# schoppmp/linreg-mpc

Measured on AMD Instinct MI355X. Metric: AND-gates/sec (garble+eval) d=500 CGD-15; phase1+2 wall-clock, higher is better.
Workload: dtype int64; 1 GPU; d=500 CGD-15 64-bit p=56, two-party masked input, garbler+evaluator co-located; one system per GPU; d=500, width=64, precision=56

## Files before the change

include/linreg_gc_debug.h:

```cpp
#ifndef LINREG_GC_DEBUG_H
#define LINREG_GC_DEBUG_H
#include "linreg_gc.h"

#ifdef __cplusplus
extern "C" {
#endif

const char *lgc_version(void);
void lgc_trace_set_tag(const char *tag);
void lgc_trace_mark(const char *what);

int lgc_device_warm(int device);
int lgc_preload(int device, int what);

int lgc_solver_get_profile(lgc_solver *s, double *garble_s, double *eval_s, size_t n);

typedef struct {
    uint32_t op, cnt, dst, a, b, c;
    int32_t sa, sb;
    uint64_t step0;
} lgc_record;
typedef struct {
    uint32_t first_rec, nrec;
    uint64_t step0, steps, gates;
    int mac_only;
} lgc_launch;
typedef struct {
    size_t n_records, n_launches;
    uint32_t n_words, n_reveal, in_base, rv_beta, rv_trace, rv_inputs;
    uint64_t total_steps, total_gates, max_launch_steps;
    uint32_t replicas, word_stride, reveal_stride;
    uint32_t shared_end, prefix_launches;
    uint64_t prefix_steps;
    uint64_t total_xors;
} lgc_program_info;
typedef struct lgc_program lgc_program;
int lgc_program_build(lgc_program **out, const lgc_system *sys);
int lgc_program_build_sweep(lgc_program **out, const lgc_system *sys, size_t count, const double *lambdas);
int lgc_program_build_sweep_at(lgc_program **out, const lgc_system *sys, size_t count, const double *lambdas, size_t first);
void lgc_program_destroy(lgc_program *p);
int lgc_program_info_get(const lgc_program *p, lgc_program_info *info);
const lgc_record *lgc_program_records(const lgc_program *p);
const lgc_launch *lgc_program_launches(const lgc_program *p);
int lgc_program_ring_plan(const lgc_program *p, size_t ring_bytes, size_t *ring_bytes_out, size_t *offsets, int64_t *wait_for);

int lgc_reference_gate_count(int algorithm, int width, size_t d, int iterations, uint64_t *gates);

int lgc_solve(int device, const lgc_system *sys, const uint8_t seed[16], const uint64_t *shares,
              int64_t *beta, int64_t *trace, lgc_stats *stats);

int lgc_party_ring_create(lgc_party *p, int nslots, uint8_t handle_out[64], size_t *slot_bytes);
int lgc_party_ring_open(lgc_party *p, const uint8_t handle[64], int nslots, size_t slot_bytes);
int lgc_party_garble_ring_streams(lgc_party *p, int streams);
void lgc_release_cached_memory(void);

void lgc_set_split_kernels(int garbler, int evaluator);

void lgc_set_karatsuba(int on);
void lgc_set_table_ring_slack(size_t bytes);

int lgc_gate_hash_eval(int device, const uint8_t *labels, const uint64_t *tweaks, uint8_t *out, size_t n);

typedef struct {
    uint8_t label[16];
    uint64_t tweak0, stride;
    uint32_t rows, reserved;
} lgc_row_item;
int lgc_row_hash_eval(int device, const lgc_row_item *items, size_t n, uint8_t *out);

int lgc_test_party_garble_ring_stage(lgc_party *p, size_t launch, int stage, int *is_critical_path);
int lgc_test_party_ring_read(lgc_party *p, size_t launch, uint8_t *out, size_t bytes);

#define LGC_LM_AUTO 0
#define LGC_LM_MAC 1
#define LGC_LM_MACK 2
#define LGC_LM_WIDE 3
#define LGC_LM_SPLIT 4
#define LGC_LM_QUAD2 5
int lgc_test_program_create(lgc_program **out, int width, int precision, const lgc_record *records, size_t n_records,
                            const uint32_t *launch_nrec, size_t n_launches, const int *mode_g, const int *mode_e,
                            uint32_t n_inputs, uint32_t n_words, uint32_t n_reveal);
int lgc_test_launch_modes(const lgc_program *p, int *mode_g, int *mode_e, size_t n);
int lgc_test_launch_shape(int mode, int garbler, uint32_t nrec, uint32_t cus, uint32_t *grid, uint32_t *threads,
                          uint32_t *per_wg, uint32_t *max_threads);
typedef struct {
    uint32_t wide_launch, narrow_mac, split_max_recs;
    uint32_t mac_chunk, mac_adapt_lo;
} lgc_test_constants;
void lgc_test_launch_constants(lgc_test_constants *c);
int lgc_test_solver_create(lgc_solver **out, int device, const lgc_program *program, const uint8_t seed[16]);
int lgc_test_solver_reveal(lgc_solver *s, uint64_t *out, size_t n);
int lgc_test_solver_read_words(lgc_solver *s, int garbler, uint32_t first, uint32_t n, uint8_t *out);
int lgc_test_solver_read_tables(lgc_solver *s, size_t launch, uint8_t *out, size_t bytes);

int lgc_test_p1_scan_block(lgc_p1 *h, size_t c0, size_t c1, size_t s0, size_t s1, int with_y, int use_rect, uint64_t *out, double *ms);

int lgc_aes_bench(int device, int waves, int blocks_per_lane, double *rate, uint32_t *check);
int lgc_aes_encrypt(int device, const uint8_t *in, uint8_t *out, size_t n);

#ifdef __cplusplus
}
#endif
#endif
```

linreg-mpc_amd/csrc/gc_engine.hip:

```cpp
#include <hip/hip_runtime.h>
#include <stdarg.h>
#include <stdio.h>
#include <stdlib.h>
#include <string.h>
#include <time.h>

#include <mutex>
#include <string>
#include <utility>
#include <vector>

#include "../../include/linreg_gc.h"
#include "../../include/linreg_gc_sweep.h"
#include "../../include/linreg_gc_debug.h"
#include "../../include/linreg_gc_targets.h"
#include "../../include/linreg_gc_lasso.h"
#include "../../include/linreg_gc_lasso_path.h"
#include "../../include/linreg_gc_lasso_opts.h"
#include "../../include/linreg_gc_lasso_select.h"
#include "../../include/linreg_gc_lasso_cv.h"
#include "../../include/linreg_gc_lasso_cv_se.h"
#include "../../include/linreg_gc_ridge_cv.h"
#include "../../include/linreg_gc_inference.h"
#include "../../include/linreg_gc_scan.h"
// ... 402 lines not shown
                            (size_t)sys->nshares, (unsigned long long)IN, r.scan);
    }
    return LGC_OK;
}

static int validate_path(const BuildRequest &r) {
    if (!r.l1) return lgc_fail(LGC_EINVAL, "null values: a lasso path needs its values of lambda1");
    if (r.l1_count < 1 || r.l1_count > LGC_MAX_L1_PATH)
        return lgc_fail(LGC_EINVAL, "a lasso path takes 1..%d values of lambda1 (got %zu)", LGC_MAX_L1_PATH, r.l1_count);
    if (r.l1_mode != LGC_L1_ABSOLUTE && r.l1_mode != LGC_L1_RATIO)
        return lgc_fail(LGC_EINVAL, "unknown lambda1 mode %d: LGC_L1_ABSOLUTE (0) or LGC_L1_RATIO (1)", r.l1_mode);
    for (size_t l = 0; l < r.l1_count; l++) {
        const double v = r.l1[l];
        if (!std::isfinite(v) || v < 0) return lgc_fail(LGC_EINVAL, "lambda1 path value %zu must be finite and >= 0 (got %g)", l, v);
        if (r.l1_mode == LGC_L1_RATIO && v > 2) return lgc_fail(LGC_EINVAL, "lambda1 ratio %zu is %g: ratios of lambda_max lie in [0, 2]", l, v);
        if (r.l1_mode == LGC_L1_RATIO && r.sys && r.sys->precision >= 0 && r.sys->precision < r.sys->width &&
            std::ldexp(v, r.sys->precision) >= std::ldexp(1.0, r.sys->width - 1))
            return lgc_fail(LGC_EINVAL, "lambda1 ratio %zu is %g: precision %d cannot hold it in a %d-bit word", l, v, r.sys->precision, r.sys->width);
    }
    if (r.sys && r.sys->trace && r.l1_count > 1)
        return lgc_fail(LGC_EINVAL, "trace is for a single lambda1 (its layout has one x per iteration)");
    return LGC_OK;
}

static bool fits_word(double v, int p, int w) {
    const double t = std::ldexp(v, p), top = std::ldexp(1.0, w - 1);
    return t >= -top && t < top;
}

static int validate_opts(const BuildRequest &r) {
    const lgc_lasso_opts &o = *r.opts;
    const int p = r.sys->precision, w = r.sys->width;
    const size_t d = (size_t)r.sys->d;
    for (size_t i = 0; i < d; i++) {
        const double f = o.penalty_factors ? o.penalty_factors[i] : 1.0;
        if (!std::isfinite(f) || f < 0) return lgc_fail(LGC_EINVAL, "penalty factor %zu must be finite and >= 0 (got %g)", i, f);
        const double lo = o.lower ? o.lower[i] : -INFINITY, hi = o.upper ? o.upper[i] : INFINITY;
        if (std::isnan(lo) || std::isnan(hi)) return lgc_fail(LGC_EINVAL, "bound %zu is NaN", i);
        if (lo == INFINITY || hi == -INFINITY)
            return lgc_fail(LGC_EINVAL, "bounds of coordinate %zu are [%g, %g]: no value lies in them", i, lo, hi);
        if (lo > hi) return lgc_fail(LGC_EINVAL, "lower bound %zu is %g, above its upper bound %g", i, lo, hi);
        for (const double v : {lo, hi})
            if (std::isfinite(v) && !fits_word(v, p, w))
                return lgc_fail(LGC_EINVAL, "bound %zu is %g: precision %d cannot hold it in a %d-bit word", i, v, p, w);
        if (!o.penalty_factors) continue;
        for (size_t l = 0; l < r.l1_count; l++) {
            const double v = r.l1[l] * f;
            if (r.l1_mode == LGC_L1_RATIO && !(std::ldexp(v, p) < std::ldexp(1.0, w - 1)))
                return lgc_fail(LGC_EINVAL, "lambda1 ratio %zu times penalty factor %zu is %g: precision %d cannot hold it in a %d-bit word",
                                l, i, v, p, w);
            if (r.l1_mode == LGC_L1_ABSOLUTE && !fits_word(v, p, w))
                return lgc_fail(LGC_EINVAL, "lambda1 %zu times penalty factor %zu is %g: precision %d cannot hold it in a %d-bit word",
                                l, i, v, p, w);
        }
    }
    return LGC_OK;
}

static uint64_t lambda_to_fixed(double lambda, int p, int w) {
    double t = lambda * (double)(1ll << p);
    if (w == 32) {
        if (!(t > -2147483649.0 && t < 2147483648.0)) return (uint64_t)(uint32_t)INT32_MIN;
        return (uint64_t)(uint32_t)(int32_t)t;
    }
    if (!(t >= -9223372036854775808.0 && t < 9223372036854775808.0)) return (uint64_t)INT64_MIN;
    return (uint64_t)(int64_t)t;
}

static int lower(Program &P, const BuildRequest &r, uint64_t cap_steps, size_t merge_hint) {
    const lgc_system *sys = r.sys;
    if (cap_steps) P.cap_steps = cap_steps;
    P.merge_hint = merge_hint;
    const int iters = (sys->algorithm == LGC_ALG_CGD || sys->algorithm == LGC_ALG_LASSO) ? sys->num_iterations : 0;
    Spec s = {sys->algorithm, sys->width, sys->precision, iters, sys->d, sys->nshares, r.targets,
              sys->normalize, sys->reveal_inputs, sys->trace,
              lambda_to_fixed(sys->lambda, sys->precision, sys->width), lambda_to_fixed(r.l1 ? *r.l1 : 0.0, sys->precision, sys->width)};
    std::vector<uint64_t> path;
    if (r.l1_mode != -1) {
        for (size_t l = 0; l < r.l1_count; l++) path.push_back(lambda_to_fixed(r.l1[l], sys->precision, sys->width));
        s.l1_mode = r.l1_mode == LGC_L1_RATIO ? L1_RATIO : L1_ABSOLUTE;
        s.l1_count = r.l1_count;
        s.l1_path = path.data();
    }
    std::vector<uint64_t> coord, lo, hi;
    std::vector<uint8_t> boxed;
    if (r.opts) {
        const lgc_lasso_opts &o = *r.opts;
        const size_t d = (size_t)sys->d;
        bool any = false;
        for (size_t i = 0; i < d; i++)
            any |= (o.penalty_factors && o.penalty_factors[i] != 1.0) || (o.lower && std::isfinite(o.lower[i])) ||
                   (o.upper && std::isfinite(o.upper[i]));
        if (any) {
            const uint64_t wmin = sys->width == 64 ? (uint64_t)INT64_MIN : (uint64_t)(uint32_t)INT32_MIN;
            const uint64_t wmax = sys->width == 64 ? (uint64_t)INT64_MAX : (uint64_t)INT32_MAX;
            for (size_t l = 0; l < r.l1_count; l++)
                for (size_t i = 0; i < d; i++)
                    coord.push_back(lambda_to_fixed(r.l1[l] * (o.penalty_factors ? o.penalty_factors[i] : 1.0), sys->precision, sys->width));
            for (size_t i = 0; i < d; i++) {
                const double a = o.lower ? o.lower[i] : -INFINITY, b = o.upper ? o.upper[i] : INFINITY;
                boxed.push_back(std::isfinite(a) || std::isfinite(b));
                lo.push_back(std::isfinite(a) ? lambda_to_fixed(a, sys->precision, sys->width) : wmin);
                hi.push_back(std::isfinite(b) ? lambda_to_fixed(b, sys->precision, sys->width) : wmax);
            }
            s.l1_coord = coord.data(); s.lo = lo.data(); s.hi = hi.data(); s.boxed = boxed.data();
        }
    }
    s.validate = r.select;
    s.select_reveal = r.reveal;
    s.folds = r.cv ? r.folds : 0;
    s.yy = r.cv && r.se;
    s.cv_rule = s.yy ? r.rule : CV_RULE_MIN;
    if (r.infer) { s.infer = r.reveal; s.resid_fixed = lambda_to_fixed(r.resid_scale, sys->precision, sys->width); }
    if (r.is_scan) {
        s.scan = r.scan; s.scan_bits = r.reveal;
        if (r.reveal & LGC_SCAN_SE) s.resid_fixed = lambda_to_fixed(r.resid_scale, sys->precision, sys->width);
    }
    build_program(P, s);
    if (r.is_scan && P.overflow) return lgc_fail(LGC_EINVAL, "scan too large: the lowered program needs more than 2^31 words");
    if (r.cv && P.overflow) return lgc_fail(LGC_EINVAL, "cross-validation too large: the lowered program needs more than 2^31 words");
    if (r.infer && P.overflow) return lgc_fail(LGC_EINVAL, "inference too large: the lowered program needs more than 2^31 words");
    if (!P.ranges_ok()) return lgc_fail(LGC_EINVAL, "internal: a record of the lowered program lies outside its word file");
    return LGC_OK;
}

static int build_ridge(Program &P, const BuildRequest &r) {
    const lgc_system *sys = r.sys;
    Spec s = {sys->algorithm, sys->width, sys->precision, sys->algorithm == LGC_ALG_CGD ? sys->num_iterations : 0, (size_t)sys->d, (size_t)sys->nshares, 1,
              sys->normalize, 0, 0, 0, 0};
    s.select_reveal = r.reveal;
    std::vector<uint64_t> lf(r.count);
    for (size_t l = 0; l < r.count; l++) lf[l] = lambda_to_fixed(r.lambdas[l], sys->precision, sys->width);
    const int rc = build_ridge_cv(P, s, r.folds, r.count, lf.data(), r.cap_steps);
    if (rc == 1) return lgc_fail(LGC_EINVAL, "ridge cross-validation too large: the lowered program needs more than 2^31 words");
    if (rc) return lgc_fail(LGC_EINVAL, "ridge cross-validation too large: its circuits (more than 65535, or one of more than 2^36 gate steps) do not fit the gate-id stride of a sweep");
    if (!P.ranges_ok()) return lgc_fail(LGC_EINVAL, "internal: a record of the ridge cross-validation lies outside its word file");
    return LGC_OK;
}
static int build(Program &P, const BuildRequest &r) {
    if (r.ridge_cv) return build_ridge(P, r);
    if (!r.sweep) return lower(P, r, r.cap_steps, 1);
    Program base;
    int rcb = lower(base, r, r.cap_steps ? r.cap_steps : kSweepCapSteps, r.count);
    if (rcb) return rcb;
    const size_t count = r.count;
    if ((uint64_t)base.n_words * count >= (1ull << 31)) return lgc_fail(LGC_EINVAL, "sweep too large: %zu circuits x %u words", count, base.n_words);
    std::vector<uint64_t> lf(count);
    for (size_t t = 0; t < count; t++) lf[t] = lambda_to_fixed(r.lambdas[t], r.sys->precision, r.sys->width);
    if (!replicate_program(P, base, count, lf.data(), r.first))
        return lgc_fail(LGC_EINVAL, "sweep too large: a circuit of %llu gate steps (or circuit index %zu) does not fit the gate-id stride of a sweep",
                        (unsigned long long)(base.total_steps - base.prefix_steps), r.first + count);
    if (!P.ranges_ok()) return lgc_fail(LGC_EINVAL, "internal: a record of the merged program lies outside its word file");
    return LGC_OK;
}

static int program_build(lgc_program **out, const BuildRequest &r) {
    int rc = validate(r);
    if (rc) return rc;
    if (!out) return lgc_fail(LGC_EINVAL, r.sweep ? "null argument" : "null out");
    lgc_program *p = new lgc_program();
    rc = build(p->P, r);
    if (rc) { delete p; return rc; }
    *out = p;
    return LGC_OK;
}
static BuildRequest sweep_request(const lgc_system *sys, size_t count, const double *lambdas, size_t first) {
    BuildRequest r = {sys};
    r.sweep = true; r.count = count; r.lambdas = lambdas; r.first = first;
    return r;
}
extern "C" int lgc_program_build(lgc_program **out, const lgc_system *sys) { return program_build(out, {sys}); }
extern "C" int lgc_program_build_lasso(lgc_program **out, const lgc_system *sys, double l1) { return program_build(out, {sys, 1, &l1}); }
static BuildRequest path_request(const lgc_system *sys, size_t count, const double *values, int mode) {
    BuildRequest r = {sys, 1, values};
    r.l1_mode = mode; r.l1_count = count;
    return r;
}
extern "C" int lgc_program_build_lasso_path(lgc_program **out, const lgc_system *sys, size_t count, const double *values, int mode) {
    return program_build(out, path_request(sys, count, values, mode));
}
static BuildRequest opts_request(const lgc_system *sys, const lgc_lasso_opts *opts) {
    BuildRequest r = path_request(sys, opts->l1_count, opts->l1, opts->l1_mode);
    r.opts = opts;
    return r;
}
extern "C" int lgc_program_build_lasso_opts(lgc_program **out, const lgc_system *sys, const lgc_lasso_opts *opts) {
    if (!opts) return lgc_fail(LGC_EINVAL, "null opts");
    return program_build(out, opts_request(sys, opts));
}
static_assert(LGC_SELECT_REVEAL_INDEX == SELECT_REVEAL_INDEX && LGC_SELECT_REVEAL_SCORES == SELECT_REVEAL_SCORES, "LGC_SELECT_REVEAL_* must name the lowering's bits");
static BuildRequest select_request(const lgc_system *sys, const lgc_lasso_opts *opts, int reveal) {
    BuildRequest r = opts_request(sys, opts);
    r.select = true; r.reveal = reveal;
    return r;
}
extern "C" int lgc_program_build_lasso_select(lgc_program **out, const lgc_system *sys, const lgc_lasso_opts *opts, int reveal) {
    if (!opts) return lgc_fail(LGC_EINVAL, "null opts");
    return program_build(out, select_request(sys, opts, reveal));
}
static BuildRequest cv_request(const lgc_system *sys, const lgc_lasso_opts *opts, size_t folds, int reveal) {
    BuildRequest r = opts_request(sys, opts);
    r.cv = true; r.folds = folds; r.reveal = reveal;
    return r;
}
extern "C" int lgc_program_build_lasso_cv(lgc_program **out, const lgc_system *sys, const lgc_lasso_opts *opts, size_t folds, int reveal) {
    if (!opts) return lgc_fail(LGC_EINVAL, "null opts");
    return program_build(out, cv_request(sys, opts, folds, reveal));
}
static_assert(LGC_SELECT_REVEAL_CURVE == SELECT_REVEAL_CURVE && LGC_CV_RULE_MIN == CV_RULE_MIN && LGC_CV_RULE_ONE_SE == CV_RULE_ONE_SE,
              "LGC_SELECT_REVEAL_CURVE and LGC_CV_RULE_* must name the lowering's values");
static BuildRequest cv_se_request(const lgc_system *sys, const lgc_lasso_opts *opts, size_t folds, int reveal, int rule) {
    BuildRequest r = cv_request(sys, opts, folds, reveal);
    r.se = true; r.rule = rule;
    return r;
}
extern "C" int lgc_program_build_lasso_cv_se(lgc_program **out, const lgc_system *sys, const lgc_lasso_opts *opts, size_t folds, int reveal,
                                             int rule) {
    if (!opts) return lgc_fail(LGC_EINVAL, "null opts");
    return program_build(out, cv_se_request(sys, opts, folds, reveal, rule));
}
static BuildRequest ridge_cv_request(const lgc_system *sys, size_t count, const double *lambdas, size_t folds, int reveal) {
    BuildRequest r = {sys};
    r.ridge_cv = true; r.count = count; r.lambdas = lambdas; r.folds = folds; r.reveal = reveal;
    return r;
}
extern "C" int lgc_program_build_ridge_cv(lgc_program **out, const lgc_system *sys, size_t count, const double *lambdas, size_t folds, int reveal) {
    return program_build(out, ridge_cv_request(sys, count, lambdas, folds, reveal));
}
static_assert(LGC_INFER_SE == INFER_SE && LGC_INFER_FIT == INFER_FIT, "LGC_INFER_* must name the lowering's bits");
static BuildRequest inference_request(const lgc_system *sys, double resid_scale, int reveal) {
    BuildRequest r = {sys};
    r.infer = true; r.resid_scale = resid_scale; r.reveal = reveal;
    return r;
}
extern "C" int lgc_program_build_inference(lgc_program **out, const lgc_system *sys, double resid_scale, int reveal) {
    return program_build(out, inference_request(sys, resid_scale, reveal));
}
static_assert(LGC_SCAN_SE == SCAN_SE, "LGC_SCAN_SE must name the lowering's bit");
static BuildRequest scan_request(const lgc_system *sys, size_t M, double resid_scale, int reveal) {
    BuildRequest r = {sys};
    r.is_scan = true; r.scan = M; r.resid_scale = resid_scale; r.reveal = reveal;
    return r;
}
extern "C" int lgc_program_build_scan(lgc_program **out, const lgc_system *sys, size_t M, double resid_scale, int reveal) {
    return program_build(out, scan_request(sys, M, resid_scale, reveal));
}
extern "C" int lgc_program_build_targets(lgc_program **out, const lgc_system *sys, size_t k) { return program_build(out, {sys, k}); }
extern "C" int lgc_program_build_sweep_at(lgc_program **out, const lgc_system *sys, size_t count, const double *lambdas, size_t first) {
    return program_build(out, sweep_request(sys, count, lambdas, first));
}
extern "C" int lgc_program_build_sweep(lgc_program **out, const lgc_system *sys, size_t count, const double *lambdas) {
    return program_build(out, sweep_request(sys, count, lambdas, 0));
}
extern "C" int lgc_program_ring_plan(const lgc_program *p, size_t ring_bytes, size_t *ring_bytes_out, size_t *offsets, int64_t *wait_for) {
    if (!p || !offsets || !wait_for) return lgc_fail(LGC_EINVAL, "null argument");
    std::vector<size_t> off;
    std::vector<int64_t> wait;
    size_t rb = plan_table_ring(p->P, ring_bytes, off, wait);
    if (ring_bytes_out) *ring_bytes_out = rb;
    for (size_t i = 0; i < off.size(); i++) { offsets[i] = off[i]; wait_for[i] = wait[i]; }
    return LGC_OK;
}
extern "C" void lgc_program_destroy(lgc_program *p) { delete p; }
extern "C" int lgc_program_info_get(const lgc_program *p, lgc_program_info *info) {
    if (!p || !info) return lgc_fail(LGC_EINVAL, "null argument");
    const Program &P = p->P;
    info->n_records = P.recs.size();
    info->n_launches = P.launches.size();
    info->n_words = P.n_words;
    info->n_reveal = P.n_reveal;
    info->in_base = P.in_base;
    info->rv_beta = P.rv_beta;
    info->rv_trace = P.rv_trace;
    info->rv_inputs = P.rv_ab;
    info->total_steps = P.total_steps;
    info->total_gates = P.total_gates;
    info->max_launch_steps = P.max_launch_steps;
    info->replicas = P.replicas;
    info->word_stride = P.word_stride;
    info->reveal_stride = P.reveal_stride;
    info->shared_end = P.shared_end;
    info->prefix_launches = P.prefix_launches;
    info->prefix_steps = P.prefix_steps;
    info->total_xors = P.total_xors;
    return LGC_OK;
}
static_assert(sizeof(lgc_record) == sizeof(Rec), "record layout");
extern "C" const lgc_record *lgc_program_records(const lgc_program *p) {
    return reinterpret_cast<const lgc_record *>(p->P.recs.data());
}
extern "C" const lgc_launch *lgc_program_launches(const lgc_program *cp) {
    lgc_program *p = const_cast<lgc_program *>(cp);
    std::vector<lgc_launch> &g_launch_tmp = p->launch_view;
    g_launch_tmp.resize(p->P.launches.size());
    for (size_t i = 0; i < g_launch_tmp.size(); i++) {
        const Launch &L = p->P.launches[i];
        lgc_launch o = {L.first_rec, L.nrec, L.step0, L.steps, L.gates, L.mac_only ? 1 : 0};
        g_launch_tmp[i] = o;
    }
    return g_launch_tmp.data();
}

static_assert(LGC_LM_AUTO == LM_NONE && LGC_LM_MAC == LM_MAC && LGC_LM_MACK == LM_MACK && LGC_LM_WIDE == LM_WIDE &&
              LGC_LM_SPLIT == LM_SPLIT && LGC_LM_QUAD2 == LM_QUAD2, "LGC_LM_* must name the LaunchMode values");
struct FootprintMachine : PlainBackend {
    uint64_t word_end = 0, slot_end = 0;
    void see(uint32_t id) { if ((uint64_t)id + 1 > word_end) word_end = (uint64_t)id + 1; }
    W load(uint32_t id) { see(id); return 0x5a5a5a5a5a5a5a5aull; }
    W load2(uint32_t lo, uint32_t hi) { see(lo); see(hi); return 0x5a5a5a5a5a5a5a5aull; }
    W load2h(uint32_t lo, uint32_t hi) { see(lo); see(hi); return 0x5a5a5a5a5a5a5a5aull; }
    W load2s(uint32_t lo, uint32_t hi, bool) { see(lo); see(hi); return 0x5a5a5a5a5a5a5a5aull; }
    void store(uint32_t id, W) { see(id); }
    void store2(uint32_t lo, uint32_t hi, W) { see(lo); see(hi); }
    void reveal(uint32_t slot, W) { if ((uint64_t)slot + 1 > slot_end) slot_end = (uint64_t)slot + 1; }
};
static bool mode_pairs_steps(LaunchMode m) { return m == LM_SPLIT || m == LM_QUAD2; }
static const char *mode_name(int m) {
    static const char *const n[] = {"auto", "MAC", "MACK", "WIDE", "SPLIT", "QUAD2"};
    return m >= 0 && m <= LM_QUAD2 ? n[m] : "?";
}

extern "C" int lgc_test_program_create(lgc_program **out, int width, int precision, const lgc_record *records, size_t n_records,
                                       const uint32_t *launch_nrec, size_t n_launches, const int *mode_g, const int *mode_e,
                                       uint32_t n_inputs, uint32_t n_words, uint32_t n_reveal) {
    if (!out || !records || !launch_nrec) return lgc_fail(LGC_EINVAL, "null argument");
    if (width != 32 && width != 64) return lgc_fail(LGC_EINVAL, "width must be 32 or 64");
    if (precision < 0 || precision >= width) return lgc_fail(LGC_EINVAL, "precision must satisfy 0 <= p < width");
    if (n_records < 1 || n_launches < 1) return lgc_fail(LGC_EINVAL, "a test program needs at least one launch and one record");
    if (n_words > (1u << 22)) return lgc_fail(LGC_EINVAL, "n_words %u above the test limit of %u", n_words, 1u << 22);
    if ((uint64_t)n_inputs + 1 > n_words) return lgc_fail(LGC_EINVAL, "%u input words at word 1 do not fit n_words = %u", n_inputs, n_words);
    uint64_t sum = 0;
    for (size_t i = 0; i < n_launches; i++) {
        if (launch_nrec[i] < 1) return lgc_fail(LGC_EINVAL, "launch %zu has no records", i);
        sum += launch_nrec[i];
    }
    if (sum != n_records) return lgc_fail(LGC_EINVAL, "the launches hold %llu records, not n_records = %zu", (unsigned long long)sum, n_records);
    for (size_t i = 0; i < n_launches; i++)
        for (int role = 0; role < 2; role++) {
            const int m = role ? (mode_e ? mode_e[i] : 0) : (mode_g ? mode_g[i] : 0);
            if (m < LGC_LM_AUTO || m > LGC_LM_QUAD2) return lgc_fail(LGC_EINVAL, "launch %zu: unknown kernel %d", i, m);
        }
    const Rec *recs = reinterpret_cast<const Rec *>(records);
    for (size_t i = 0; i < n_records; i++) {
        const Rec &r = recs[i];
        if (r.op >= OP_COUNT_) return lgc_fail(LGC_EINVAL, "record %zu: op %u is not an op (OP_COUNT_ = %u)", i, r.op, (unsigned)OP_COUNT_);
        if (width == 64 && r.op == OP_MAC2) return lgc_fail(LGC_EINVAL, "record %zu: OP_MAC2 is a 32-bit op", i);
        if (width == 32 && (r.op == OP_MACK || r.op == OP_HDIFF || r.op == OP_DIVB))
            return lgc_fail(LGC_EINVAL, "record %zu: op %u is a 64-bit op", i, r.op);
        FootprintMachine fm;
        exec_record(fm, r, width, precision);
        if (fm.word_end > n_words)
            return lgc_fail(LGC_EINVAL, "record %zu (op %u): touches word %llu, outside n_words = %u", i, r.op,
                            (unsigned long long)(fm.word_end - 1), n_words);
        if (fm.slot_end > n_reveal)
            return lgc_fail(LGC_EINVAL, "record %zu (op %u): reveals to slot %llu, outside n_reveal = %u", i, r.op,
                            (unsigned long long)(fm.slot_end - 1), n_reveal);
    }
    lgc_program *p = new lgc_program();
    Program &P = p->P;
    P.w = width; P.p = precision;
    P.d = 0; P.T = n_inputs; P.nshares = 1;
    P.in_base = 1; P.shared_end = 1;
    P.n_words = n_words; P.n_reveal = n_reveal;
    size_t next = 0;
    for (size_t i = 0; i < n_launches; i++) {
        P.new_launch();
        for (uint32_t k = 0; k < launch_nrec[i]; k++) P.emit(recs[next++]);
        if (P.launches.size() != i + 1) {
            delete p;
            return lgc_fail(LGC_EINVAL, "launch %zu mixes MAC records (OP_MAC / OP_MAC2 / OP_MACK) with others or with each other, or "
                                        "exceeds the table cap: the lowering would split it", i);
        }
    }
    for (size_t i = 0; i < n_launches; i++) {
        Launch &L = P.launches[i];
        L.force[0] = (uint8_t)(mode_g ? mode_g[i] : 0);
        L.force[1] = (uint8_t)(mode_e ? mode_e[i] : 0);
        for (int role = 0; role < 2; role++) {
            const int m = L.force[role];
            if ((m == LM_MAC || m == LM_MACK) && !L.mac_only) {
                delete p;
                return lgc_fail(LGC_EINVAL, "launch %zu: the %s kernel runs MAC-only launches", i, mode_name(m));
            }
            if ((m == LM_MAC && L.mack) || (m == LM_MACK && !L.mack)) {
                delete p;
                return lgc_fail(LGC_EINVAL, "launch %zu: the %s kernel cannot run %s records", i, mode_name(m),
                                L.mack ? "OP_MACK" : "OP_MAC / OP_MAC2");
            }
        }
        const LaunchMode g = gc_launch_mode(L, true), e = gc_launch_mode(L, false);
        if (mode_pairs_steps(g) != mode_pairs_steps(e)) {
            delete p;
            return lgc_fail(LGC_EINVAL, "launch %zu: garbler %s and evaluator %s number the gate steps differently (kPairSteps)", i,
                            mode_name(g), mode_name(e));
        }
    }
    if (!P.ranges_ok()) {
        delete p;
        return lgc_fail(LGC_EINVAL, "internal: a record of the test program lies outside its word file");
    }
    *out = p;
    return LGC_OK;
}
extern "C" int lgc_test_launch_modes(const lgc_program *p, int *mode_g, int *mode_e, size_t n) {
    if (!p || !mode_g || !mode_e) return lgc_fail(LGC_EINVAL, "null argument");
    if (n != p->P.launches.size()) return lgc_fail(LGC_EINVAL, "n must equal the number of launches (%zu)", p->P.launches.size());
    for (size_t i = 0; i < n; i++) {
        mode_g[i] = gc_launch_mode(p->P.launches[i], true);
        mode_e[i] = gc_launch_mode(p->P.launches[i], false);
    }
    return LGC_OK;
}
extern "C" int lgc_test_launch_shape(int mode, int garbler, uint32_t nrec, uint32_t cus, uint32_t *grid, uint32_t *threads,
                                     uint32_t *per_wg, uint32_t *max_threads) {
    if (!grid || !threads || !per_wg || !max_threads) return lgc_fail(LGC_EINVAL, "null argument");
    if (mode < LGC_LM_MAC || mode > LGC_LM_QUAD2) return lgc_fail(LGC_EINVAL, "unknown kernel %d", mode);
    if (cus < 1) return lgc_fail(LGC_EINVAL, "cus must be >= 1");
    const LaunchShape sh = gc_launch_shape((LaunchMode)mode, garbler != 0, nrec, cus);
    *grid = sh.grid; *threads = sh.threads; *per_wg = sh.per_wg;
    switch (mode) {
    case LM_MAC: *max_threads = garbler ? kTpbMacG : kTpbMacE; break;
    case LM_MACK: *max_threads = garbler ? kTpbMackG : kTpbMackE; break;
    case LM_WIDE: *max_threads = kTpbWide; break;
    case LM_SPLIT: *max_threads = 1024; break;
    default: *max_threads = 256; break;
    }
    return LGC_OK;
}
extern "C" void lgc_test_launch_constants(lgc_test_constants *c) {
    c->wide_launch = kWideLaunch;
    c->narrow_mac = kNarrowMac;
    c->split_max_recs = kSplitMaxRecs;
    c->mac_chunk = kMacChunk;
    c->mac_adapt_lo = kMacAdaptLo;
}

struct lgc_solver {
    lgc_system sys;
    Program P;
    int device;
    Lbl R, seed;
    Lbl *wordsG, *wordsE, *tab;
    uint64_t *decG, *decE, *vals;
    Rec *recs;
    hipStream_t stream, streamE, streamT;
    hipEvent_t ev0, ev1, ev_in;
    size_t ring_bytes;
    size_t tab_alloc_bytes;
    std::vector<size_t> tab_off;
    std::vector<int64_t> tab_wait;
    std::vector<hipEvent_t> evG, evE;
    std::vector<hipEvent_t> evC;
    std::vector<hipEvent_t> evs;
    std::vector<uint64_t> hG, hE;
    std::vector<double> tG, tE;
    std::vector<hipEvent_t> ev_iter;
    std::vector<double> t_iter;
    bool have_shares, ran;
    bool prefix_ready;
    bool prefix_imported = false;
    lgc_stats st;
    lgc_solver() : wordsG(0), wordsE(0), tab(0), decG(0), decE(0), vals(0), recs(0), stream(0), streamE(0), streamT(0), ev0(0), ev1(0), ev_in(0), ring_bytes(0), tab_alloc_bytes(0),
                   have_shares(false), ran(false), prefix_ready(false) { memset(&st, 0, sizeof(st)); }
};

namespace {
struct RingCache {
    std::mutex mu;
    struct Slot { int device; void *ptr; size_t bytes; };
    std::vector<Slot> slots;
    void *take(int device, size_t need, size_t *bytes) {
        std::lock_guard<std::mutex> g(mu);
        for (size_t i = 0; i < slots.size(); i++)
            if (slots[i].device == device && slots[i].bytes >= need) {
                void *p = slots[i].ptr;
                *bytes = slots[i].bytes;
                slots.erase(slots.begin() + (long)i);
                return p;
            }
        return 0;
    }
    void park(int device, void *ptr, size_t bytes) {
        std::lock_guard<std::mutex> g(mu);
        for (size_t i = 0; i < slots.size(); i++)
            if (slots[i].device == device) {
                if (slots[i].bytes >= bytes) { (void)hipFree(ptr); return; }
                (void)hipFree(slots[i].ptr);
                slots[i].ptr = ptr; slots[i].bytes = bytes;
                return;
            }
        Slot n = {device, ptr, bytes};
        slots.push_back(n);
    }
    void release(int device) {
        std::lock_guard<std::mutex> g(mu);
        for (size_t i = 0; i < slots.size();) {
            if (device < 0 || slots[i].device == device) {
                (void)hipSetDevice(slots[i].device);
                (void)hipFree(slots[i].ptr);
                slots.erase(slots.begin() + (long)i);
            } else {
                i++;
            }
        }
    }
};
RingCache &ring_cache() { static RingCache c; return c; }
}

extern "C" void lgc_release_cached_memory(void) { ring_cache().release(-1); }

extern "C" void lgc_solver_destroy(lgc_solver *s) {
    if (!s) return;
    (void)hipSetDevice(s->device);
    if (s->wordsG) (void)hipFree(s->wordsG);
    if (s->wordsE) (void)hipFree(s->wordsE);
    if (s->tab) {
        (void)hipDeviceSynchronize();
        ring_cache().park(s->device, s->tab, s->tab_alloc_bytes);
    }
    if (s->decG) (void)hipFree(s->decG);
    if (s->decE) (void)hipFree(s->decE);
    if (s->vals) (void)hipFree(s->vals);
    if (s->recs) (void)hipFree(s->recs);
    for (size_t i = 0; i < s->evs.size(); i++) (void)hipEventDestroy(s->evs[i]);
    for (size_t i = 0; i < s->ev_iter.size(); i++) (void)hipEventDestroy(s->ev_iter[i]);
    if (s->ev0) (void)hipEventDestroy(s->ev0);
    if (s->ev1) (void)hipEventDestroy(s->ev1);
    for (size_t i = 0; i < s->evG.size(); i++) (void)hipEventDestroy(s->evG[i]);
    for (size_t i = 0; i < s->evE.size(); i++) (void)hipEventDestroy(s->evE[i]);
    for (size_t i = 0; i < s->evC.size(); i++) (void)hipEventDestroy(s->evC[i]);
    if (s->ev_in) (void)hipEventDestroy(s->ev_in);
    if (s->stream) (void)hipStreamDestroy(s->stream);
    if (s->streamE) (void)hipStreamDestroy(s->streamE);
    if (s->streamT) (void)hipStreamDestroy(s->streamT);
    delete s;
}

static int solver_alloc(lgc_solver *s, const uint8_t seed[16], lgc_solver **out);
static int solver_create(lgc_solver **out, int device, const uint8_t seed[16], const BuildRequest &r) {
    int rc = validate(r);
    if (rc) return rc;
    if (!out || !seed) return lgc_fail(LGC_EINVAL, "null argument");
    rc = lgc_need_device(device);
    if (rc) return rc;
    lgc_solver *s = new lgc_solver();
    s->sys = *r.sys;
    s->device = device;
    rc = build(s->P, r);
    if (rc) { delete s; return rc; }
    return solver_alloc(s, seed, out);
}
static int solver_alloc(lgc_solver *s, const uint8_t seed[16], lgc_solver **out) {
    memcpy(&s->seed, seed, 16);
    s->R = derive_R(s->seed);
    const Program &P = s->P;
    size_t wbytes = (size_t)P.n_words * 64 * sizeof(Lbl);
    size_t nin = P.nshares * P.in_words();
#define TRY(x)                                                                                   \
    do {                                                                                         \
        hipError_t e_ = (x);                                                                     \
        if (e_ != hipSuccess) {                                                                  \
            lgc_fail(e_ == hipErrorOutOfMemory ? LGC_ENOMEM : LGC_EHIP, "%s: %s", #x, hipGetErrorString(e_)); \
            lgc_solver_destroy(s);                                                               \
            return e_ == hipErrorOutOfMemory ? LGC_ENOMEM : LGC_EHIP;                            \
        }                                                                                        \
    } while (0)
    TRY(hipStreamCreate(&s->stream));
    TRY(hipStreamCreate(&s->streamE));
    TRY(hipStreamCreate(&s->streamT));
    TRY(hipEventCreate(&s->ev0));
    TRY(hipEventCreate(&s->ev1));
    TRY(hipEventCreateWithFlags(&s->ev_in, hipEventDisableTiming));
    s->ring_bytes = plan_table_ring(P, 0, s->tab_off, s->tab_wait);
    TRY(hipMalloc(&s->wordsG, wbytes));
    TRY(hipMalloc(&s->wordsE, wbytes));
    s->tab = reinterpret_cast<Lbl *>(ring_cache().take(s->device, s->ring_bytes, &s->tab_alloc_bytes));
    if (!s->tab) {
        hipError_t em = hipMalloc(&s->tab, s->ring_bytes);
        if (em == hipErrorOutOfMemory) {
            (void)hipGetLastError();
            ring_cache().release(s->device);
            em = hipMalloc(&s->tab, s->ring_bytes);
        }
        TRY(em);
        s->tab_alloc_bytes = s->ring_bytes;
    }
    TRY(hipMalloc(&s->decG, (P.n_reveal + 1) * sizeof(uint64_t)));
    TRY(hipMalloc(&s->decE, (P.n_reveal + 1) * sizeof(uint64_t)));
    TRY(hipMalloc(&s->vals, nin * sizeof(uint64_t)));
    TRY(hipMalloc(&s->recs, P.recs.size() * sizeof(Rec)));
    TRY(hipMemcpy(s->recs, P.recs.data(), P.recs.size() * sizeof(Rec), hipMemcpyHostToDevice));
#undef TRY
    s->hG.resize(P.n_reveal + 1);
    s->hE.resize(P.n_reveal + 1);
    *out = s;
    return LGC_OK;
}
extern "C" int lgc_solver_create(lgc_solver **out, int device, const lgc_system *sys, const uint8_t seed[16]) {
    return solver_create(out, device, seed, {sys});
}
extern "C" int lgc_solver_create_sweep_at(lgc_solver **out, int device, const lgc_system *sys, const uint8_t seed[16],
                                          size_t count, const double *lambdas, size_t first) {
    return solver_create(out, device, seed, sweep_request(sys, count, lambdas, first));
}
extern "C" int lgc_solver_create_sweep(lgc_solver **out, int device, const lgc_system *sys, const uint8_t seed[16],
                                       size_t count, const double *lambdas) {
    return solver_create(out, device, seed, sweep_request(sys, count, lambdas, 0));
}
extern "C" size_t lgc_solver_num_circuits(const lgc_solver *s) { return s ? (s->P.ridge_cv ? s->P.path : s->P.replicas) : 0; }
extern "C" int lgc_solver_create_ridge_cv(lgc_solver **out, int device, const lgc_system *sys, const uint8_t seed[16], size_t count,
                                          const double *lambdas, size_t folds, int reveal) {
    return solver_create(out, device, seed, ridge_cv_request(sys, count, lambdas, folds, reveal));
}
extern "C" int lgc_solver_create_inference(lgc_solver **out, int device, const lgc_system *sys, const uint8_t seed[16], double resid_scale, int reveal) {
    return solver_create(out, device, seed, inference_request(sys, resid_scale, reveal));
}
extern "C" int lgc_solver_create_scan(lgc_solver **out, int device, const lgc_system *sys, const uint8_t seed[16], size_t M, double resid_scale, int reveal) {
    return solver_create(out, device, seed, scan_request(sys, M, resid_scale, reveal));
}
extern "C" int lgc_solver_create_targets(lgc_solver **out, int device, const lgc_system *sys, const uint8_t seed[16], size_t k) {
    return solver_create(out, device, seed, {sys, k});
}
extern "C" size_t lgc_solver_num_targets(const lgc_solver *s) { return s ? s->P.targets : 0; }
extern "C" int lgc_solver_create_lasso(lgc_solver **out, int device, const lgc_system *sys, const uint8_t seed[16], double l1) {
    return solver_create(out, device, seed, {sys, 1, &l1});
}
extern "C" int lgc_solver_create_lasso_path(lgc_solver **out, int device, const lgc_system *sys, const uint8_t seed[16], size_t count,
                                            const double *values, int mode) {
    return solver_create(out, device, seed, path_request(sys, count, values, mode));
}
extern "C" int lgc_solver_create_lasso_opts(lgc_solver **out, int device, const lgc_system *sys, const uint8_t seed[16],
                                            const lgc_lasso_opts *opts) {
    if (!opts) return lgc_fail(LGC_EINVAL, "null opts");
    return solver_create(out, device, seed, opts_request(sys, opts));
}
extern "C" int lgc_solver_create_lasso_select(lgc_solver **out, int device, const lgc_system *sys, const uint8_t seed[16],
                                              const lgc_lasso_opts *opts, int reveal) {
    if (!opts) return lgc_fail(LGC_EINVAL, "null opts");
    return solver_create(out, device, seed, select_request(sys, opts, reveal));
}
extern "C" int lgc_solver_create_lasso_cv(lgc_solver **out, int device, const lgc_system *sys, const uint8_t seed[16],
                                          const lgc_lasso_opts *opts, size_t folds, int reveal) {
    if (!opts) return lgc_fail(LGC_EINVAL, "null opts");
    return solver_create(out, device, seed, cv_request(sys, opts, folds, reveal));
}
extern "C" int lgc_solver_create_lasso_cv_se(lgc_solver **out, int device, const lgc_system *sys, const uint8_t seed[16],
                                             const lgc_lasso_opts *opts, size_t folds, int reveal, int rule) {
    if (!opts) return lgc_fail(LGC_EINVAL, "null opts");
    return solver_create(out, device, seed, cv_se_request(sys, opts, folds, reveal, rule));
}
extern "C" size_t lgc_solver_num_folds(const lgc_solver *s) { return s ? s->P.folds : 0; }
extern "C" size_t lgc_solver_path_length(const lgc_solver *s) { return s ? s->P.path : 0; }

extern "C" int lgc_test_solver_create(lgc_solver **out, int device, const lgc_program *program, const uint8_t seed[16]) {
    if (!out || !program || !seed) return lgc_fail(LGC_EINVAL, "null argument");
    const int rc = lgc_need_device(device);
    if (rc) return rc;
    lgc_solver *s = new lgc_solver();
    memset(&s->sys, 0, sizeof(s->sys));
    s->sys.width = program->P.w;
    s->sys.precision = program->P.p;
    s->sys.nshares = program->P.nshares;
    s->device = device;
    s->P = program->P;
    return solver_alloc(s, seed, out);
}
extern "C" int lgc_test_solver_reveal(lgc_solver *s, uint64_t *out, size_t n) {
    if (!s || !out) return lgc_fail(LGC_EINVAL, "null argument");
    if (!s->ran) return lgc_fail(LGC_ESTATE, "solver has not run");
    if (n != s->P.n_reveal) return lgc_fail(LGC_EINVAL, "n must equal n_reveal (%u)", s->P.n_reveal);
    const uint64_t m = s->P.w == 64 ? ~0ull : (1ull << s->P.w) - 1;
    for (size_t i = 0; i < n; i++) out[i] = (s->hG[i] ^ s->hE[i]) & m;
    return LGC_OK;
}

extern "C" int lgc_test_solver_read_words(lgc_solver *s, int garbler, uint32_t first, uint32_t n, uint8_t *out) {
    if (!s || !out) return lgc_fail(LGC_EINVAL, "null argument");
    if (!s->ran) return lgc_fail(LGC_ESTATE, "solver has not run");
    if ((uint64_t)first + n > s->P.n_words) return lgc_fail(LGC_EINVAL, "words [%u, %u + %u) lie outside the word file (%u words)", first, first, n, s->P.n_words);
    HIPCHK(hipSetDevice(s->device));
    HIPCHK(hipMemcpy(out, (garbler ? s->wordsG : s->wordsE) + (size_t)first * 64, (size_t)n * 64 * sizeof(Lbl), hipMemcpyDeviceToHost));
    return LGC_OK;
}
extern "C" int lgc_test_solver_read_tables(lgc_solver *s, size_t launch, uint8_t *out, size_t bytes) {
    if (!s || !out) return lgc_fail(LGC_EINVAL, "null argument");
    if (!s->ran) return lgc_fail(LGC_ESTATE, "solver has not run");
    const Program &P = s->P;
    if (launch >= P.launches.size() || bytes != (size_t)P.launches[launch].steps * 2048)
        return lgc_fail(LGC_EINVAL, "launch out of range, or bytes is not 2048 x its gate steps");
    for (size_t k = launch + 1; k < P.launches.size(); k++) {
        const size_t kb = (size_t)P.launches[k].steps * 2048;
        if (kb && s->tab_off[k] < s->tab_off[launch] + bytes && s->tab_off[launch] < s->tab_off[k] + kb)
            return lgc_fail(LGC_ESTATE, "launch %zu has reused the ring region of launch %zu", k, launch);
    }
    HIPCHK(hipSetDevice(s->device));
    HIPCHK(hipMemcpy(out, reinterpret_cast<const uint8_t *>(s->tab) + s->tab_off[launch], bytes, hipMemcpyDeviceToHost));
    return LGC_OK;
}

extern "C" int lgc_solver_set_shares(lgc_solver *s, const uint64_t *shares) {
    if (!s || !shares) return lgc_fail(LGC_EINVAL, "null argument");
    HIPCHK(hipSetDevice(s->device));
    size_t nin = s->P.nshares * s->P.in_words();
    HIPCHK(hipMemcpy(s->vals, shares, nin * sizeof(uint64_t), hipMemcpyHostToDevice));
    s->have_shares = true;
    return LGC_OK;
}

extern "C" int lgc_solver_run(lgc_solver *s, int profile) {
    if (!s) return lgc_fail(LGC_EINVAL, "null solver");
    if (!s->have_shares && !s->prefix_ready)
        return lgc_fail(LGC_ESTATE, s->prefix_imported ? "the imported prefix has been consumed: import again before the next run"
                                                       : "lgc_solver_set_shares has not been called");
    HIPCHK(hipSetDevice(s->device));
    const Program &P = s->P;
    size_t wbytes = (size_t)P.n_words * 64 * sizeof(Lbl);
    size_t nin = P.nshares * P.in_words();
    const size_t nl = P.launches.size();
    size_t need_ev = 3 * nl;
    while (s->evs.size() < need_ev) {
        hipEvent_t e;
        HIPCHK(hipEventCreate(&e));
        s->evs.push_back(e);
    }
    while (s->evG.size() < nl) {
        hipEvent_t a, b;
        HIPCHK(hipEventCreateWithFlags(&a, hipEventDisableTiming));
        s->evG.push_back(a);
        HIPCHK(hipEventCreateWithFlags(&b, hipEventDisableTiming));
        s->evE.push_back(b);
        HIPCHK(hipEventCreateWithFlags(&b, hipEventDisableTiming));
        s->evC.push_back(b);
    }
    hipStream_t sG = s->stream, sE = profile ? s->stream : s->streamE;
// ... 373 lines not shown
```

linreg-mpc_amd/csrc/gc_kernels.h:

```cpp
#pragma once
#include <hip/hip_runtime.h>

#include "gc_device.h"
#include "gc_split.h"
#include "gc_launch.h"

namespace gc {

static inline hipError_t gc_launch_tabfill_impl(const Launch &L, const Lbl *stash, Lbl *tab, Lbl R, hipStream_t st) {
    const uint64_t per = kTpbTabfill / 64;
    uint64_t blocks = (L.steps + per - 1) / per;
    if (blocks > 2048) blocks = 2048;
    hipLaunchKernelGGL((gc_tabfill_kernel<kTpbTabfill>), dim3((unsigned)blocks), dim3(kTpbTabfill), 0, st, stash, tab,
                       (uint32_t)L.steps, L.step0, R);
    return hipGetLastError();
}

template <bool G, int PART>
static inline hipError_t gc_launch_records_impl(LaunchMode m, const Rec *recs, const Launch &L, Lbl *words, uint64_t *dec, Lbl *tab, Lbl R, int w,
                                    int p, hipStream_t st) {
    switch (m) {
    case LM_NONE:
        return hipSuccess;
    case LM_MAC: if constexpr (PART == 0) {
        constexpr int TPB = G ? kTpbMacG : kTpbMacE;
        const LaunchShape sh = gc_launch_shape(m, G, L.nrec, gc_num_cus());
        hipLaunchKernelGGL((gc_mac_kernel<G, TPB>), dim3(sh.grid), dim3(sh.threads), 0, st, recs + L.first_rec, L.nrec, sh.per_wg,
                           words, tab, L.step0, R, w, p);
    } break;
    case LM_MACK: if constexpr (PART == 0) {
        constexpr int TPB = G ? kTpbMackG : kTpbMackE;
        const LaunchShape sh = gc_launch_shape(m, G, L.nrec, gc_num_cus());
        hipLaunchKernelGGL((gc_mack_kernel<G, TPB>), dim3(sh.grid), dim3(sh.threads), 0, st,
                           recs + L.first_rec, L.nrec, sh.per_wg, words, tab, L.step0, R, w, p);
    } break;
    case LM_WIDE: if constexpr (PART == 1) {
        const LaunchShape sh = gc_launch_shape(m, G, L.nrec, gc_num_cus());
        hipLaunchKernelGGL((gc_exec_kernel<G, false, 4, kTpbWide>), dim3(sh.grid), dim3(sh.threads), 0, st,
                           recs + L.first_rec, L.nrec, words, tab, dec, L.step0, R, w, p);
    } break;
    case LM_SPLIT:
        if constexpr (PART == 2) {
            const LaunchShape sh = gc_launch_shape(m, G, L.nrec, gc_num_cus());
            hipLaunchKernelGGL((gc_split_kernel<G>), dim3(sh.grid), dim3(sh.threads), 0, st, recs + L.first_rec, L.nrec, words, tab, dec,
                               L.step0, R, w, p);
        }
        break;
    case LM_QUAD2:
        if constexpr (PART == 3) {
            const LaunchShape sh = gc_launch_shape(m, G, L.nrec, gc_num_cus());
            hipLaunchKernelGGL((gc_exec_kernel<G, true, 2, 256>), dim3(sh.grid), dim3(sh.threads), 0, st, recs + L.first_rec, L.nrec, words,
                               tab, dec, L.step0, R, w, p);
        }
        break;
    }
    return hipGetLastError();
}

}
```

linreg-mpc_amd/csrc/gc_launch.h:

```cpp
#pragma once
#include <hip/hip_runtime.h>

#include <atomic>
#include <cstdlib>
#include <vector>

#include "gc_aes.h"
#include "gc_program.h"

namespace gc {

#ifndef GC_TPB_MACG
#define GC_TPB_MACG 1024
#endif
#ifndef GC_TPB_MACE
#define GC_TPB_MACE 768
#endif
#ifndef GC_TPB_MACKG
#define GC_TPB_MACKG 1024
#endif
#ifndef GC_TPB_MACKE
#define GC_TPB_MACKE 768
#endif
static constexpr int kTpbMacG = GC_TPB_MACG, kTpbMacE = GC_TPB_MACE, kTpbMackG = GC_TPB_MACKG, kTpbMackE = GC_TPB_MACKE;
#ifndef GC_WIDE_LAUNCH
#define GC_WIDE_LAUNCH 520
#endif
static constexpr uint32_t kWideLaunch = GC_WIDE_LAUNCH;
static constexpr int kTpbWide = 768;
static constexpr uint32_t kNarrowMac = 1024;
static constexpr uint32_t kExclusiveMac = 4096;
static constexpr int kTpbTabfill = 1024;
#ifndef GC_SPLIT_MAX_RECS
#define GC_SPLIT_MAX_RECS 256
#endif
static constexpr uint32_t kSplitMaxRecs = GC_SPLIT_MAX_RECS;
inline std::atomic<int> &gc_split_enabled(bool garbler) {
    static std::atomic<int> on[2] = {{1}, {1}};
    return on[garbler ? 0 : 1];
}

static inline unsigned gc_num_cus() {
    static int cus = 0;
    if (!cus) {
        int dev = 0;
        hipDeviceProp_t prop;
        if (hipGetDevice(&dev) == hipSuccess && hipGetDeviceProperties(&prop, dev) == hipSuccess && prop.multiProcessorCount > 0)
            cus = prop.multiProcessorCount;
        else
            cus = 256;
    }
    return (unsigned)cus;
}
static constexpr unsigned kMacAdaptLo = 12, kMacAdaptMaxRounds = 8, kMackAdaptMaxRounds = 3;
static inline unsigned gc_adapt_waves(uint32_t nrec, unsigned lo, unsigned hi, unsigned max_rounds, uint64_t cus) {
    if (((uint64_t)nrec + hi - 1) / hi > (uint64_t)max_rounds * cus || nrec <= cus * lo) return hi;
    unsigned best = hi;
    uint64_t best_cost = ~0ull;
    for (unsigned wv = hi; wv >= lo; wv--) {
        uint64_t wgs = (nrec + wv - 1) / wv, rounds = (wgs + cus - 1) / cus, cost = rounds * wv;
        if (cost < best_cost) { best_cost = cost; best = wv; }
    }
    return best;
}
static constexpr unsigned kMacChunk = 32, kMacChunkMinRounds = 1;
static inline unsigned gc_mac_per_wg(uint32_t nrec, unsigned waves, uint64_t cus) {
    if ((uint64_t)nrec < (uint64_t)kMacChunkMinRounds * cus * waves) return waves;
    uint64_t rounds = ((uint64_t)nrec + cus * waves * kMacChunk / 2) / (cus * waves * kMacChunk);
    if (rounds < 1) rounds = 1;
    const uint64_t wgs = rounds * cus;
    return (unsigned)(((uint64_t)nrec + wgs - 1) / wgs);
}

enum LaunchMode {
    LM_NONE = 0,
    LM_MAC,
    LM_MACK,
    LM_WIDE,
    LM_SPLIT,
    LM_QUAD2
};
static_assert(LM_QUAD2 < 256, "Launch::force holds a LaunchMode in a byte");
static inline LaunchMode gc_launch_mode(const Launch &L, bool garbler) {
    if (L.nrec == 0) return LM_NONE;
    if (L.force[garbler ? 0 : 1]) return (LaunchMode)L.force[garbler ? 0 : 1];
    if (L.mac_only && L.nrec >= kNarrowMac) return L.mack ? LM_MACK : LM_MAC;
    if (L.nrec >= kWideLaunch) return LM_WIDE;
    if (L.nrec <= kSplitMaxRecs && gc_split_enabled(garbler).load(std::memory_order_relaxed)) return LM_SPLIT;
    return LM_QUAD2;
}
struct LaunchShape { uint32_t grid, threads, per_wg; };
static inline LaunchShape gc_launch_shape(LaunchMode m, bool garbler, uint32_t nrec, uint64_t cus) {
    LaunchShape s = {0u, 0u, 0u};
    switch (m) {
    case LM_MAC:
    case LM_MACK: {
        const unsigned tpb = m == LM_MAC ? (garbler ? kTpbMacG : kTpbMacE) : (garbler ? kTpbMackG : kTpbMackE);
        const unsigned per = gc_adapt_waves(nrec, kMacAdaptLo, tpb / 64, m == LM_MAC ? kMacAdaptMaxRounds : kMackAdaptMaxRounds, cus);
        s.per_wg = gc_mac_per_wg(nrec, per, cus);
        s.threads = per * 64;
    } break;
    case LM_WIDE: {
        uint64_t per = ((uint64_t)nrec + cus - 1) / cus;
        if (per > (uint64_t)kTpbWide / 64) per = kTpbWide / 64;
        s.per_wg = (uint32_t)per;
        s.threads = s.per_wg * 64;
    } break;
    case LM_SPLIT: s.per_wg = 1; s.threads = 1024; break;
    case LM_QUAD2: s.per_wg = 1; s.threads = 256; break;
    default: return s;
    }
    s.grid = (uint32_t)(((uint64_t)nrec + s.per_wg - 1) / s.per_wg);
    return s;
}
static inline bool gc_mode_is_crit(LaunchMode m, const Launch &L) { return L.steps != 0 && m == LM_SPLIT; }
hipError_t gc_launch_tabfill(const Launch &L, const Lbl *stash, Lbl *tab, Lbl R, hipStream_t st);
#define GC_KERN_DECL(tag)                                                                                                              \
    hipError_t gc_launch_records_##tag(LaunchMode m, const Rec *recs, const Launch &L, Lbl *words, uint64_t *dec, Lbl *tab, Lbl R, int w, \
                                       int p, hipStream_t st);                                                                         \
    hipError_t gc_kern_touch_##tag(hipStream_t st);
GC_KERN_DECL(g_0) GC_KERN_DECL(g_1) GC_KERN_DECL(g_2) GC_KERN_DECL(g_3) GC_KERN_DECL(e_0) GC_KERN_DECL(e_1) GC_KERN_DECL(e_2) GC_KERN_DECL(e_3)
#undef GC_KERN_DECL
template <bool G>
static inline hipError_t gc_launch_records(LaunchMode m, const Rec *recs, const Launch &L, Lbl *words, uint64_t *dec, Lbl *tab, Lbl R,
                                          int w, int p, hipStream_t st) {
    switch (m) {
    case LM_NONE: return hipSuccess;
    case LM_MAC: case LM_MACK: return G ? gc_launch_records_g_0(m, recs, L, words, dec, tab, R, w, p, st) : gc_launch_records_e_0(m, recs, L, words, dec, tab, R, w, p, st);
    case LM_SPLIT: return G ? gc_launch_records_g_2(m, recs, L, words, dec, tab, R, w, p, st) : gc_launch_records_e_2(m, recs, L, words, dec, tab, R, w, p, st);
    case LM_WIDE: return G ? gc_launch_records_g_1(m, recs, L, words, dec, tab, R, w, p, st) : gc_launch_records_e_1(m, recs, L, words, dec, tab, R, w, p, st);
    default: return G ? gc_launch_records_g_3(m, recs, L, words, dec, tab, R, w, p, st) : gc_launch_records_e_3(m, recs, L, words, dec, tab, R, w, p, st);
    }
}

template <bool G>
static hipError_t gc_preload(const std::vector<Launch> &launches, hipStream_t st) {
    bool need[4] = {false, false, false, false};
    for (const Launch &L : launches) {
        switch (gc_launch_mode(L, G)) {
        case LM_NONE: break;
        case LM_MAC: case LM_MACK: need[0] = true; break;
        case LM_WIDE: need[1] = true; break;
        case LM_SPLIT: need[2] = true; break;
        default: need[3] = true; break;
        }
    }
    hipError_t e = hipSuccess;
    if (need[0] && e == hipSuccess) e = G ? gc_kern_touch_g_0(st) : gc_kern_touch_e_0(st);
    if (need[1] && e == hipSuccess) e = G ? gc_kern_touch_g_1(st) : gc_kern_touch_e_1(st);
    if (need[2] && e == hipSuccess) e = G ? gc_kern_touch_g_2(st) : gc_kern_touch_e_2(st);
    if (need[3] && e == hipSuccess) e = G ? gc_kern_touch_g_3(st) : gc_kern_touch_e_3(st);
    return e;
}

template <bool G>
static hipError_t gc_launch(const Rec *recs, const Launch &L, Lbl *words, uint64_t *dec, Lbl *tab, Lbl R, int w, int p,
                            hipStream_t st, Lbl *stash = 0, int stages = 3, bool *was_crit = 0) {
    const LaunchMode m = gc_launch_mode(L, G);
    const bool crit = G && gc_mode_is_crit(m, L);
    if (was_crit) *was_crit = crit;
    Lbl *rec_tab = (crit && stash) ? stash : tab;
    hipError_t e = hipSuccess;
    if (stages & 1) e = gc_launch_records<G>(m, recs, L, words, dec, rec_tab, R, w, p, st);
    if (e == hipSuccess && crit && (stages & 2)) e = gc_launch_tabfill(L, rec_tab, tab, R, st);
    return e;
}

}
```

linreg-mpc_amd/csrc/gc_split.h:

```cpp
#pragma once
#include "gc_device.h"

namespace gc {

template <int CTRL> __device__ __forceinline__ uint32_t quad_perm(uint32_t v) {
    return (uint32_t)__builtin_amdgcn_mov_dpp((int)v, CTRL, 0xf, 0xf, true);
}

struct HashNoHook { __device__ __forceinline__ void operator()(int) const {} };
template <class F = HashNoHook>
__device__ __forceinline__ uint32_t hash_split(const LdsTab4 &lt, const uint32_t rkl[11], uint32_t x, uint32_t twc, int c, F beside = F()) {
    const uint32_t t = quad_perm<0x4E>(x);
    const uint32_t k = (c < 2) ? (t ^ twc) : (x ^ t);
    uint32_t s = k ^ rkl[0];
#pragma unroll
    for (int rnd = 1; rnd < 10; rnd++) {
        const uint32_t s1 = quad_perm<0x39>(s), s2 = quad_perm<0x4E>(s), s3 = quad_perm<0x93>(s);
        const uint32_t v0 = lt.lkt(0, s, 0), v1 = lt.lkt(1, s1, 1), v2 = lt.lkt(2, s2, 2), v3 = lt.lkt(3, s3, 3);
        beside(rnd);
        s = xor3(xor3(v0, v1, rkl[rnd]), v2, v3);
    }
    const uint32_t s1 = quad_perm<0x39>(s), s2 = quad_perm<0x4E>(s), s3 = quad_perm<0x93>(s);
    const uint32_t v0 = lt.lk(s, 0), v1 = lt.lk(s1, 1), v2 = lt.lk(s2, 2), v3 = lt.lk(s3, 3);
    s = xor3(last_lo(v1, v0), last_hi(v3, v2), rkl[10]);
    return s ^ k;
}

enum {
    kSplitPlane = 72,
    kSplitWord = 4 * kSplitPlane,
    kSplitOp = 0,
    kSplitX = 4 * kSplitWord,
    kSplitKs = 8 * kSplitWord,
    kSplitGs = 16 * kSplitWord,
    kSplitDesc = 20 * kSplitWord,
    kSplitZero = 20 * kSplitWord + 8,
    kSplitWords = 20 * kSplitWord + 16
};

struct SplitDesc {
    uint32_t kind;
    uint64_t act1, act2;
    uint64_t step;
};

struct SplitHashCtx {
    LdsTab4 lt;
    uint32_t rkl[11];
    uint32_t Rq;
    uint32_t *sx;
    __attribute__((address_space(3))) uint32_t *sxl;
    uint32_t *tabw;
    uint64_t launch_step0;
    int wave, lane;
};

__device__ __forceinline__ uint32_t rfl(uint32_t v) { return (uint32_t)__builtin_amdgcn_readfirstlane((int)v); }
__device__ __forceinline__ void st_u32_global(uint32_t *p, uint32_t v) { *(__attribute__((address_space(1))) uint32_t *)p = v; }
__device__ __forceinline__ uint32_t ld_u32_global(const uint32_t *p) { return *(const __attribute__((address_space(1))) uint32_t *)p; }
__device__ __forceinline__ void st_u32_lds(uint32_t *p, uint32_t v) { *(__attribute__((address_space(3))) uint32_t *)p = v; }
__device__ __forceinline__ uint32_t ld_u32_lds(const uint32_t *p) { return *(const __attribute__((address_space(3))) uint32_t *)p; }

__device__ __forceinline__ uint32_t *split_row(const SplitHashCtx &hc, int q, uint64_t st) {
    const int gate = 16 * (hc.wave & 3) + (hc.lane >> 2);
    return hc.tabw + ((st - hc.launch_step0) * 128 + (uint64_t)((q & 1) * 64 + gate)) * 4 + (hc.lane & 3);
}
template <bool GARBLER>
__device__ __forceinline__ void split_hash_core(const SplitHashCtx &hc, int q, uint64_t act, uint64_t st, uint32_t a_op, uint32_t b_op,
                                                uint32_t *xdst, uint32_t tg) {
    const int r = hc.wave & 3, c = hc.lane & 3, gate = 16 * r + (hc.lane >> 2);
    uint32_t *row = split_row(hc, q, st);
    uint32_t *xo = xdst + c * kSplitPlane + gate;
    const uint32_t act16 = (uint32_t)(act >> (16 * r)) & 0xffffu;
    if (act16 == 0) {
        st_u32_lds(xo, 0u);
        if (GARBLER) st_u32_global(row, 0u);
        return;
    }
    const bool on = (act16 >> (hc.lane >> 2)) & 1u;
    const uint32_t v = (q & 1) ? b_op : a_op;
    if (GARBLER) st_u32_global(row, on ? v : 0u);
    const uint32_t colour = quad_perm<0x00>(v) & 1u;
    const uint32_t x = GARBLER ? (v ^ (colour ? hc.Rq : 0u)) : v;
    const uint32_t tlo = ((uint32_t)st << 7) | (uint32_t)(2 * gate + (q & 1)), thi = (uint32_t)(st >> 25);
    const uint32_t twc = (c == 0) ? tlo : (c == 1) ? thi : 0u;
    uint32_t h = hash_split(hc.lt, hc.rkl, x, twc, c);
    if (GARBLER) {
        if (!(q & 1)) h ^= (colour & quad_perm<0x00>(b_op) & 1u) ? hc.Rq : 0u;
    } else {
        h ^= colour ? ((q & 1) ? (tg ^ a_op) : tg) : 0u;
    }
    st_u32_lds(xo, on ? h : 0u);
}

template <bool GARBLER>
__device__ __forceinline__ void split_hash_phase(const SplitHashCtx &hc, const SplitDesc &d) {
    const int q = hc.wave >> 2, r = hc.wave & 3;
    if (d.kind == 1 && q >= 2) return;
    const int c = hc.lane & 3, gate = 16 * r + (hc.lane >> 2);
    const uint32_t *op = hc.sx + kSplitOp + c * kSplitPlane + gate;
    const uint32_t a_op = ld_u32_lds(op + (q & ~1) * kSplitWord), b_op = ld_u32_lds(op + (q | 1) * kSplitWord);
    const uint64_t st = d.step + (uint64_t)(q >> 1);
    const uint32_t tg = GARBLER ? 0u : ld_u32_global(split_row(hc, q, st));
    split_hash_core<GARBLER>(hc, q, (q < 2) ? d.act1 : d.act2, st, a_op, b_op, hc.sx + kSplitX + q * kSplitWord, tg);
}

#ifndef GC_SPLIT_TRACE
#define GC_SPLIT_TRACE 0
#endif
#if GC_SPLIT_TRACE
static __device__ uint64_t g_split_trace[2 * 8192];
static __device__ uint32_t g_split_trace_n[2];
struct SkTrace { bool on; int w; uint32_t i; };
#define SPLIT_STAMP(tag)                                                                                         \
    if (tr.on) {                                                                                                 \
        uint64_t t_;                                                                                             \
        asm volatile("s_memtime %0\n\ts_waitcnt lgkmcnt(0)" : "=s"(t_));                                         \
        if (hc.lane == 0 && tr.i < 8192) g_split_trace[tr.w * 8192 + tr.i] = (t_ << 4) | (uint64_t)(tag);        \
        tr.i++;                                                                                                  \
    }
#define SPLIT_STAMP2(wv, tag)                                                                                    \
    if (GC_SPLIT_TRACE == 2 && blockIdx.x == 0) {                                                                \
        uint64_t t_;                                                                                             \
        asm volatile("s_memtime %0\n\ts_waitcnt lgkmcnt(0)" : "=s"(t_));                                         \
        const uint32_t i_ = g_split_trace_n[wv];                                                                 \
        if ((threadIdx.x & 63) == 0) { if (i_ < 8192) g_split_trace[(wv) * 8192 + i_] = (t_ << 4) | (uint64_t)(tag); g_split_trace_n[wv] = i_ + 1; } \
    }
#else
struct SkTrace {};
#define SPLIT_STAMP(tag)
#define SPLIT_STAMP2(wv, tag)
#endif

typedef __attribute__((address_space(3))) uint32_t lds_u32;

struct SkPtrs {
    const lds_u32 *o0, *o1, *o2;
    const lds_u32 *p0, *p1, *p2;
};

__device__ __forceinline__ int sk_levels(int n) { return n <= 1 ? 0 : 32 - __builtin_clz((uint32_t)(n - 1)); }

__device__ __forceinline__ void sk_words_a(const lds_u32 *sx, int k, int g, int pl, const lds_u32 *&a0, const lds_u32 *&a1) {
    const lds_u32 *opx = sx + kSplitOp + pl, *opy = opx + kSplitWord, *opc = opx + 2 * kSplitWord;
    if (k < 0) { a0 = opx + g; a1 = opc + g; return; }
    const int h = 1 << k, hp = h >> 1;
    const int t = ((g >> k) & 1) ? g : ((g + h) & 63);
    if (k == 0) { a0 = opx + t; a1 = opy + t; return; }
    const lds_u32 *X0 = sx + kSplitKs + ((k & 1) * 4) * kSplitWord + pl, *X1 = X0 + kSplitWord;
    const lds_u32 *Pp = sx + kSplitGs + (((k - 1) & 1) * 2 + 1) * kSplitWord + pl;
    const bool tp = (g >> (k - 1)) & 1;
    const int ti = tp ? t - hp : t;
    a0 = (tp ? X0 : Pp) + ti;
    a1 = tp ? X1 + ti : sx + kSplitZero;
}
__device__ __forceinline__ void sk_words_b(const lds_u32 *sx, int k, int g, int pl, const lds_u32 *&b0, const lds_u32 *&b1, const lds_u32 *&b2) {
    const lds_u32 *opx = sx + kSplitOp + pl, *opy = opx + kSplitWord, *opc = opx + 2 * kSplitWord;
    const lds_u32 *zero = sx + kSplitZero;
    if (k < 0) { b0 = opy + g; b1 = opc + g; b2 = zero; return; }
    const int h = 1 << k, hp = h >> 1;
    const bool up = (g >> k) & 1;
    const int mb = (g & ~(2 * h - 1)) | (h - 1);
    const lds_u32 *X0 = sx + kSplitKs + ((k & 1) * 4) * kSplitWord + pl, *X1 = X0 + kSplitWord;
    if (k == 0) {
        b0 = (up ? X0 : opx) + mb;
        b1 = (up ? X1 : opy) + mb;
        b2 = up ? opc + mb : zero;
        return;
    }
    const lds_u32 *Gp = sx + kSplitGs + (((k - 1) & 1) * 2) * kSplitWord + pl;
    const int mi = up ? mb : ((mb - hp) & 63);
    b0 = X0 + mi;
    b1 = X1 + mi;
    b2 = up ? Gp + mb : zero;
}
template <int Q>
__device__ __forceinline__ void sk_ptrs_own(SkPtrs &r, const lds_u32 *sx, int k, int g, int pl) {
    if (Q == 0) { sk_words_a(sx, k, g, pl, r.o0, r.o1); r.o2 = sx + kSplitZero; }
    else sk_words_b(sx, k, g, pl, r.o0, r.o1, r.o2);
}
template <int Q>
__device__ __forceinline__ void sk_ptrs_oth(SkPtrs &r, const lds_u32 *sx, int k, int g, int plo) {
    if (Q == 0) sk_words_b(sx, k, g, plo, r.p0, r.p1, r.p2);
    else { sk_words_a(sx, k, g, plo, r.p0, r.p1); r.p2 = sx + kSplitZero; }
}

struct SkPlan {
    SkPtrs ptr;
    uint32_t twc;
    bool on;
    bool any;
};
__device__ __forceinline__ bool sk_gate_on(int k, int g, int n) {
    if (k < 0) return g < n;
    const int h = 1 << k;
    return ((g >> k) & 1) ? (g < n) : (g >= 2 * h && g + h < n);
}
template <bool GARBLER, int Q>
__device__ __forceinline__ void sk_plan_part(SkPlan &r, int part, const lds_u32 *sx, int k, int g, int c, int pl, int plo, int n, uint64_t st) {
    constexpr bool kNeedOth = GARBLER ? (Q == 0) : (Q == 1);
    if (part == 0) sk_ptrs_own<Q>(r.ptr, sx, k, g, pl);
    if (part == 1) { if (kNeedOth) sk_ptrs_oth<Q>(r.ptr, sx, k, g, plo); else { r.ptr.p0 = r.ptr.p1 = r.ptr.p2 = sx + kSplitZero; } }
    if (part == 2) {
        const uint32_t tlo = ((uint32_t)st << 7) | (uint32_t)(2 * g + Q), thi = (uint32_t)(st >> 25);
        r.twc = (c == 0) ? tlo : (c == 1) ? thi : 0u;
    }
    if (part == 3) {
        r.on = sk_gate_on(k, g, n);
        r.any = __builtin_amdgcn_ballot_w64(r.on) != 0ull;
    }
}
template <bool GARBLER, int Q>
__device__ __forceinline__ SkPlan sk_plan(const lds_u32 *sx, int k, int g, int c, int pl, int plo, int n, uint64_t st) {
    SkPlan r;
    for (int part = 0; part < 4; part++) sk_plan_part<GARBLER, Q>(r, part, sx, k, g, c, pl, plo, n, st);
    return r;
}

struct SkVals { uint32_t l0, l1, l2, m0, m1, m2; };
template <bool GARBLER, int Q>
__device__ __forceinline__ SkVals sk_load(const SkPtrs &ptr) {
    constexpr bool kNeedOth = GARBLER ? (Q == 0) : (Q == 1);
    SkVals v;
    v.l0 = *ptr.o0; v.l1 = *ptr.o1; v.l2 = (Q == 1) ? *ptr.o2 : 0u;
    v.m0 = v.m1 = v.m2 = 0u;
    if (kNeedOth) { v.m0 = *ptr.p0; v.m1 = *ptr.p1; v.m2 = (Q == 0) ? *ptr.p2 : 0u; }
    return v;
}
template <bool GARBLER, int Q, class F>
__device__ __forceinline__ void sk_finish(const SplitHashCtx &hc, const SkPlan &lv, const SkVals &w, lds_u32 *xo, uint32_t *row, uint32_t tg, F beside) {
    const int c = hc.lane & 3;
    const bool on = lv.on;
    const uint32_t twc = lv.twc;
    if (!lv.any) {
        *xo = 0u;
        if (GARBLER) st_u32_global(row, 0u);
        for (int rnd = 1; rnd < 10; rnd++) beside(rnd);
        return;
    }
    const uint32_t v = xor3(w.l0, w.l1, w.l2);
    if (GARBLER) st_u32_global(row, on ? v : 0u);
    const uint32_t colour = quad_perm<0x00>(v) & 1u;
    const uint32_t x = GARBLER ? (v ^ (colour ? hc.Rq : 0u)) : v;
    uint32_t h = hash_split(hc.lt, hc.rkl, x, twc, c, beside);
    if (GARBLER) {
        if (Q == 0) h ^= (colour & (w.m0 ^ w.m1 ^ w.m2) & 1u) ? hc.Rq : 0u;
    } else {
        h ^= colour ? ((Q == 1) ? (tg ^ xor3(w.m0, w.m1, w.m2)) : tg) : 0u;
    }
    *xo = on ? h : 0u;
}

template <bool GARBLER, int Q>
__device__ __forceinline__ void split_sk_hash(const SplitHashCtx &hc, int n, uint64_t st, const SkVals *pre) {
    const int r = hc.wave & 3, c = hc.lane & 3, g = 16 * r + (hc.lane >> 2);
    SkTrace tr;
    (void)tr;
#if GC_SPLIT_TRACE
    tr.on = GC_SPLIT_TRACE == 1 && blockIdx.x == 0 && (hc.wave == 0 || hc.wave == 4);
    tr.w = hc.wave == 4 ? 1 : 0;
    tr.i = tr.on ? g_split_trace_n[tr.w] : 0u;
    SPLIT_STAMP(1)
#endif
    lds_u32 *sx = hc.sxl;
    const int pl = c * kSplitPlane, plo = GARBLER ? 0 : pl;
    const int L = sk_levels(n);
    uint32_t *row = split_row(hc, Q, st);
    uint32_t tA = 0, tB = 0;
    if (!GARBLER) {
        tA = ld_u32_global(row);
        tB = ld_u32_global(row + (L > 0 ? 512 : 0));
    }
    SkPlan cur = sk_plan<GARBLER, Q>(sx, -1, g, c, pl, plo, n, st), nxt;
    SkVals w = pre ? *pre : sk_load<GARBLER, Q>(cur.ptr);
    sk_finish<GARBLER, Q>(hc, cur, w, sx + kSplitKs + Q * kSplitWord + pl + g, row, tA,
                          [&](int rnd) { if (rnd >= 2 && rnd < 6) sk_plan_part<GARBLER, Q>(nxt, rnd - 2, sx, 0, g, c, pl, plo, n, st + 1); });
    if (!GARBLER) tA = ld_u32_global(row + (L > 1 ? 2 * 512 : 0));
    st += 1;
    row += 512;
    SPLIT_STAMP(2)
    lds_barrier();
    SPLIT_STAMP(3)
    auto level = [&](int k, uint32_t &tg) {
        cur = nxt;
        w = sk_load<GARBLER, Q>(cur.ptr);
        sk_finish<GARBLER, Q>(hc, cur, w, sx + kSplitKs + (((k + 1) & 1) * 4 + Q) * kSplitWord + pl + g, row, tg,
                              [&](int rnd) { if (rnd >= 2 && rnd < 6) sk_plan_part<GARBLER, Q>(nxt, rnd - 2, sx, k + 1, g, c, pl, plo, n, st + 1); });
        if (!GARBLER) tg = ld_u32_global(row + (k + 2 < L ? 2 * 512 : 0));
        SPLIT_STAMP(5)
        st += 1;
        row += 512;
        lds_barrier();
        SPLIT_STAMP(3)
    };
    int k = 0;
    for (; k + 1 < L; k += 2) { level(k, tB); level(k + 1, tA); }
    if (k < L) level(k, tB);
#if GC_SPLIT_TRACE
    if (tr.on && hc.lane == 0) g_split_trace_n[tr.w] = tr.i < 8192 ? tr.i : 8192;
#endif
}

__device__ __forceinline__ void split_sk_side(const SplitHashCtx &hc, int n) {
    const int q = hc.wave >> 2, r = hc.wave & 3, c = hc.lane & 3, g = 16 * r + (hc.lane >> 2);
    lds_u32 *sx = hc.sxl;
    const int pl = c * kSplitPlane;
    const lds_u32 *opx = sx + kSplitOp + pl, *opy = opx + kSplitWord, *opc = opx + 2 * kSplitWord;
    const int L = sk_levels(n);
    lds_barrier();
    for (int k = 0; k < L; k++) {
        if (q == 2) {
            const int h = 1 << k, hp = h >> 1;
            const lds_u32 *X0 = sx + kSplitKs + ((k & 1) * 4) * kSplitWord + pl, *X1 = X0 + kSplitWord;
            const lds_u32 *Gp = sx + kSplitGs + (((k - 1) & 1) * 2) * kSplitWord + pl, *Pp = Gp + kSplitWord;
            lds_u32 *Go = sx + kSplitGs + ((k & 1) * 2) * kSplitWord + pl;
            const uint32_t x0 = X0[g], x1 = X1[g];
            uint32_t Gs, Ps;
            if (k == 0) {
                Gs = x0 ^ x1 ^ opc[g];
                Ps = opx[g] ^ opy[g];
            } else {
                const bool gp = ((g >> (k - 1)) & 1) && g >= h;
                const int gi = gp ? g - hp : g;
                const uint32_t p1 = (gp ? X0 : Pp)[gi], p2 = X1[gi], go = Gp[g];
                Gs = go ^ (((g >> (k - 1)) & 1) ? (x0 ^ x1) : 0u);
                Ps = gp ? (p1 ^ p2) : p1;
            }
            Go[g] = Gs;
            Go[kSplitWord + g] = Ps;
        }
        lds_barrier();
    }
}

template <bool GARBLER>
struct SplitBackend {
    typedef uint32_t W;
    static const bool kPairSteps = true;
    SplitHashCtx hc;
    uint32_t Rc;
    Lbl *words;
    uint64_t *decode;
    uint64_t step;
    int wave, lane;

    __device__ __forceinline__ W zero() const { return 0u; }
    __device__ __forceinline__ bool bit(uint64_t m) const { return __builtin_amdgcn_inverse_ballot_w64(m); }
    __device__ __forceinline__ W rmask(uint64_t m) const { return bit(m) ? Rc : 0u; }
    __device__ __forceinline__ W konst(uint64_t bits) const { return GARBLER ? rmask(bits) : 0u; }
    __device__ __forceinline__ W XOR(W a, W b) const { return a ^ b; }
    __device__ __forceinline__ W NOTm(W a, uint64_t m) const { return GARBLER ? (a ^ rmask(m)) : a; }
    __device__ __forceinline__ W sel(uint64_t m, W a, W b) const { return bit(m) ? a : b; }
    __device__ __forceinline__ W bcast(W a, int src) const { return (uint32_t)__builtin_amdgcn_readlane((int)a, src); }
    __device__ __forceinline__ W bcast2(W a, int r) const { return sel(0xffffffffull, bcast(a, r), bcast(a, 32 + r)); }
    __device__ __forceinline__ W pull(W a, int from, bool ok) const {
        uint32_t v = (uint32_t)__builtin_amdgcn_ds_bpermute((from & 63) << 2, (int)a);
        return ok ? v : 0u;
    }
    __device__ __forceinline__ W bblk(W a, int k) const { const int h = 1 << k; return pull(a, (lane & ~(2 * h - 1)) | (h - 1), true); }
    __device__ __forceinline__ W up1(W a) const { return (uint32_t)__builtin_amdgcn_update_dpp(0, (int)a, 0x138, 0xf, 0xf, true); }
    __device__ __forceinline__ W down1(W a) const { return (uint32_t)__builtin_amdgcn_update_dpp(0, (int)a, 0x130, 0xf, 0xf, true); }
    __device__ __forceinline__ W shl(W a, int k) const {
        if (k == 1) return up1(a);
        if (k == 2) return up1(up1(a));
        return k >= 64 ? 0u : pull(a, lane - k, lane >= k);
    }
    __device__ __forceinline__ W shr(W a, int k) const {
        if (k == 1) return down1(a);
        return k >= 64 ? 0u : pull(a, lane + k, lane + k < 64);
    }

    __device__ __forceinline__ const uint32_t *col(const Lbl *p) const { return reinterpret_cast<const uint32_t *>(p) + wave; }
    __device__ __forceinline__ uint32_t *col(Lbl *p) const { return reinterpret_cast<uint32_t *>(p) + wave; }
    __device__ __forceinline__ W load(uint32_t id) const { return ld_u32_global(col(words + (size_t)id * 64 + lane)); }
    __device__ __forceinline__ W load2(uint32_t lo, uint32_t hi) const {
        return ld_u32_global(col(words + (size_t)(lane < 32 ? lo : hi) * 64 + (lane & 31)));
    }
    __device__ __forceinline__ W load2h(uint32_t lo, uint32_t hi) const {
        return ld_u32_global(col(words + (size_t)(lane < 32 ? lo : hi) * 64 + 32 + (lane & 31)));
    }
    __device__ __forceinline__ W load2s(uint32_t lo, uint32_t hi, bool upper) const { return upper ? load2h(lo, hi) : load2(lo, hi); }
    __device__ __forceinline__ void store(uint32_t id, W v) { st_u32_global(col(words + (size_t)id * 64 + lane), v); }
    __device__ __forceinline__ void store2(uint32_t lo, uint32_t hi, W v) {
        st_u32_global(col(words + (size_t)(lane < 32 ? lo : hi) * 64 + (lane & 31)), v);
    }
    __device__ __forceinline__ void reveal(uint32_t slot, W v) {
        uint64_t m = __ballot(v & 1u);
        if (wave == 0 && lane == 0) decode[slot] = m;
    }

    __device__ __forceinline__ void publish(int k, W v) { st_u32_lds(hc.sx + kSplitOp + k * kSplitWord + wave * kSplitPlane + lane, v); }
    __device__ __forceinline__ W result(int q) const { return ld_u32_lds(hc.sx + kSplitX + q * kSplitWord + wave * kSplitPlane + lane); }
    __device__ __forceinline__ void post(const SplitDesc &d, int n = 0) {
        if (wave == 0 && lane == 0) {
            typedef __attribute__((address_space(3))) gc_u32x4 *lds4;
            gc_u32x4 lo = {d.kind | ((uint32_t)n << 8), (uint32_t)d.step, (uint32_t)(d.step >> 32), (uint32_t)d.act1};
            ((lds4)(hc.sx + kSplitDesc))[0] = lo;
            if (d.kind != 3u) {
                gc_u32x4 hi = {(uint32_t)(d.act1 >> 32), (uint32_t)d.act2, (uint32_t)(d.act2 >> 32), 0u};
                ((lds4)(hc.sx + kSplitDesc))[1] = hi;
            }
        }
    }
    __device__ __forceinline__ W AND(W a, W b, uint64_t act) {
        SplitDesc d = {1u, act, 0ull, step};
        step++;
        publish(0, a);
        publish(1, b);
        post(d);
        lds_barrier();
        split_hash_phase<GARBLER>(hc, d);
        lds_barrier();
        return bit(act) ? (result(0) ^ result(1)) : 0u;
    }
    __device__ __forceinline__ void AND2(W a1, W b1, uint64_t act1, W a2, W b2, uint64_t act2, W &c1, W &c2) {
        SplitDesc d = {2u, act1, act2, step};
        step += 2;
        if (wave == 0) { SPLIT_STAMP2(0, 6) }
        publish(0, a1);
        publish(1, b1);
        publish(2, a2);
        publish(3, b2);
        post(d);
        lds_barrier();
        if (wave == 0) { SPLIT_STAMP2(0, 7) }
        split_hash_phase<GARBLER>(hc, d);
        if (wave == 0) { SPLIT_STAMP2(0, 8) }
        lds_barrier();
        if (wave == 0) { SPLIT_STAMP2(0, 9) }
        c1 = bit(act1) ? (result(0) ^ result(1)) : 0u;
        c2 = bit(act2) ? (result(2) ^ result(3)) : 0u;
        if (wave == 0) { asm volatile("" :: "v"(c1), "v"(c2)); SPLIT_STAMP2(0, 10) }
    }
    __device__ __forceinline__ W add_native(W x, W y, int n, W cinw, W *cout) {
        const int L = sk_levels(n);
        SplitDesc d = {3u, 0ull, 0ull, step};
        const uint64_t st0 = step;
        step += 1 + (uint64_t)L;
        publish(0, x);
        publish(1, y);
        publish(2, cinw);
        post(d, n);
        lds_barrier();
        split_sk_hash<GARBLER, 0>(hc, n, st0, (const SkVals *)0);
        const lds_u32 *sx = hc.sxl;
        const int pl = wave * kSplitPlane;
        const lds_u32 *X0 = sx + kSplitKs + ((L & 1) * 4) * kSplitWord + pl, *X1 = X0 + kSplitWord;
        const lds_u32 *Gp = (L == 0) ? (sx + kSplitOp + 2 * kSplitWord + pl) : (sx + kSplitGs + (((L - 1) & 1) * 2) * kSplitWord + pl);
        const int tm = (lane - 1) & 63;
        const bool xm = (L == 0) || ((tm >> (L - 1)) & 1);
        const uint32_t gm = Gp[tm], x0m = X0[tm], x1m = X1[tm];
        uint32_t co = 0u;
        if (cout) {
            const bool xc = (L == 0) || (((n - 1) >> (L - 1)) & 1);
            co = Gp[n - 1] ^ (xc ? (X0[n - 1] ^ X1[n - 1]) : 0u);
        }
        const uint32_t Gsh = (lane > 0 && lane < n) ? (gm ^ (xm ? (x0m ^ x1m) : 0u)) : 0u;
        if (cout) *cout = co;
        return x ^ y ^ cinw ^ Gsh;
    }
    __device__ __forceinline__ void finish() {
        SplitDesc d = {0u, 0ull, 0ull, 0ull};
        post(d);
        lds_barrier();
    }
};

template <bool GARBLER>
__global__ void __launch_bounds__(1024)
gc_split_kernel(const Rec *recs, uint32_t nrec, Lbl *words, Lbl *tab, uint64_t *decode, uint64_t launch_step0, Lbl R, int w, int p) {
    __shared__ uint32_t lds_te0[2 * kLdsTabWords];
    __shared__ __attribute__((aligned(16))) uint32_t lds_sx[kSplitWords];
    lds_tab4_fill(lds_te0);
    const uint32_t wid = blockIdx.x;
    if (wid >= nrec) return;
    SplitHashCtx hc;
    hc.lt = lds_tab4_make(lds_te0);
    hc.lane = threadIdx.x & 63;
    hc.wave = __builtin_amdgcn_readfirstlane(threadIdx.x >> 6);
    const int c = hc.lane & 3;
#pragma unroll
    for (int k = 0; k < 11; k++) hc.rkl[k] = c_aes.rk[4 * k + c];
    hc.Rq = GARBLER ? (c == 0 ? R.x : c == 1 ? R.y : c == 2 ? R.z : R.w) : 0u;
    hc.sx = lds_sx;
    hc.sxl = (__attribute__((address_space(3))) uint32_t *)lds_sx;
    if (threadIdx.x == 0) lds_sx[kSplitZero] = 0u;
    hc.tabw = reinterpret_cast<uint32_t *>(tab);
    hc.launch_step0 = launch_step0;
    if (hc.wave >= 4) {
        const int q = hc.wave >> 2;
        const int g_ = 16 * (hc.wave & 3) + (hc.lane >> 2), pl_ = c * kSplitPlane;
        SkPtrs first1;
        sk_ptrs_own<1>(first1, hc.sxl, -1, g_, pl_);
        sk_ptrs_oth<1>(first1, hc.sxl, -1, g_, GARBLER ? 0 : pl_);
        for (;;) {
            lds_barrier();
            typedef const __attribute__((address_space(3))) gc_u32x4 *lds4;
            const gc_u32x4 lo = ((lds4)(lds_sx + kSplitDesc))[0];
            SkVals pre;
            if (q == 1) pre = sk_load<GARBLER, 1>(first1);
            SplitDesc d;
            const uint32_t kn = rfl(lo.x);
            d.kind = kn & 0xffu;
            if (d.kind == 0u) return;
            d.step = ((uint64_t)rfl(lo.z) << 32) | rfl(lo.y);
            if (d.kind == 3u) {
                const int n = (int)(kn >> 8);
                if (q == 1) split_sk_hash<GARBLER, 1>(hc, n, d.step, &pre);
                else split_sk_side(hc, n);
                continue;
            }
            const gc_u32x4 hi = ((lds4)(lds_sx + kSplitDesc))[1];
            d.act1 = ((uint64_t)rfl(hi.x) << 32) | rfl(lo.w);
            d.act2 = ((uint64_t)rfl(hi.z) << 32) | rfl(hi.y);
            if (hc.wave == 4) { SPLIT_STAMP2(1, 7) }
            split_hash_phase<GARBLER>(hc, d);
            if (hc.wave == 4) { SPLIT_STAMP2(1, 8) }
            lds_barrier();
            if (hc.wave == 4) { SPLIT_STAMP2(1, 9) }
        }
    }
    SplitBackend<GARBLER> be;
    be.hc = hc;
    be.wave = hc.wave;
    be.lane = hc.lane;
    be.Rc = GARBLER ? (hc.wave == 0 ? R.x : hc.wave == 1 ? R.y : hc.wave == 2 ? R.z : R.w) : 0u;
    be.words = words;
    be.decode = decode;
    Rec r = recs[wid];
    r.op = __builtin_amdgcn_readfirstlane(r.op);
    r.cnt = __builtin_amdgcn_readfirstlane(r.cnt);
    r.dst = __builtin_amdgcn_readfirstlane(r.dst);
    r.a = __builtin_amdgcn_readfirstlane(r.a);
    r.b = __builtin_amdgcn_readfirstlane(r.b);
    r.c = __builtin_amdgcn_readfirstlane(r.c);
    r.sa = __builtin_amdgcn_readfirstlane(r.sa);
    r.sb = __builtin_amdgcn_readfirstlane(r.sb);
    uint32_t s_lo = __builtin_amdgcn_readfirstlane((uint32_t)r.step0);
    uint32_t s_hi = __builtin_amdgcn_readfirstlane((uint32_t)(r.step0 >> 32));
    be.step = ((uint64_t)s_hi << 32) | s_lo;
    exec_record(be, r, w, p);
    be.finish();
}

}
```

linreg-mpc_amd/python/linreg_gc.py:

```python
import ctypes as C
import os
import types

import numpy as np

_HERE = os.path.dirname(os.path.abspath(__file__))
LIB_PATH = os.environ.get("LGC_LIB") or os.path.join(os.path.dirname(_HERE), "csrc", "liblinreg_gc.so")

ALG = {"cholesky": 0, "ldlt": 1, "cgd": 2, "dimcheck": 3,
       "lasso": 4}


class LgcError(RuntimeError):
    def __init__(self, code, msg):
        RuntimeError.__init__(self, "lgc error %d: %s" % (code, msg))
        self.code = code


class System(C.Structure):
    _fields_ = [("d", C.c_size_t), ("width", C.c_int), ("precision", C.c_int), ("algorithm", C.c_int),
                ("num_iterations", C.c_int), ("lam", C.c_double), ("nshares", C.c_size_t),
                ("normalize", C.c_int), ("reveal_inputs", C.c_int), ("trace", C.c_int)]


# ... 914 lines not shown
        _chk(lib().lgc_party_evaluate_ring(self._h, k))

    def garble_ring_begin(self, k):
        _chk(lib().lgc_party_garble_ring_begin(self._h, k))

    def garble_ring_streams(self, n):
        _chk(lib().lgc_party_garble_ring_streams(self._h, n))

    def garble_ring_wait(self, k):
        _chk(lib().lgc_party_garble_ring_wait(self._h, k))

    def test_garble_ring_stage(self, k, stage):
        crit = C.c_int()
        _chk(lib().lgc_test_party_garble_ring_stage(self._h, k, stage, C.byref(crit)))
        return bool(crit.value)

    def test_ring_read(self, k, nbytes):
        out = np.zeros(max(1, nbytes), dtype=np.uint8)
        _chk(lib().lgc_test_party_ring_read(self._h, k, _vp(out), nbytes))
        return out[:nbytes]

    def decode_bits(self):
        out = np.zeros(max(1, self.num_reveal), dtype=np.uint64)
        _chk(lib().lgc_party_decode_bits(self._h, _vp(out)))
        return out

    def finish(self, garbler_dec):
        out = np.zeros(self._req.revealed_shape(), dtype=np.int64)
        trace = np.zeros((1 if self.scan is not None else max(1, self.system.num_iterations), _trace_width(self.system)), dtype=np.int64)
        inputs = np.zeros(self._req.in_words(), dtype=np.int64)
        garbler_dec = np.ascontiguousarray(garbler_dec, dtype=np.uint64)
        _chk(lib().lgc_party_finish(self._h, _vp(garbler_dec), _vp(out), _vp(trace), _vp(inputs)))
        self._result = self._req.split(out)
        return self._result.beta, trace, inputs

    def _need(self, what, name):
        what = "select" if what == "curve" else what
        if self._result is None or getattr(self, what) is None:
            raise LgcError(-1, self._FOLLOWS.get(what) or "%s follows finish() of a model selection" % name)

    def _revealed(self):
        return self._result

    def close(self):
        if self._h:
            lib().lgc_party_destroy(self._h); self._h = None

    def __del__(self):
        try:
            self.close()
        except Exception:
            pass


def share_choice_bits(values, width):
    values = np.ascontiguousarray(values, dtype=np.uint64)
    return ((values[:, None] >> np.arange(width, dtype=np.uint64)[None, :]) & np.uint64(1)).astype(np.uint8).ravel()


class OtSender:

    def __init__(self, delta, seeds, device=0):
        seeds = np.ascontiguousarray(seeds, dtype=np.uint8).reshape(128, 16)
        self._h = C.c_void_p()
        _chk(lib().lgc_ot_sender_create(C.byref(self._h), device, bytes(delta), _vp(seeds)))

    def gilboa(self, b, width, u):
        b = np.ascontiguousarray(b, dtype=np.uint64); npairs, n = b.shape
        y = np.zeros(npairs * n * width, dtype=np.uint64); sh = np.zeros(npairs, dtype=np.uint64)
        _chk(lib().lgc_ot_gilboa_send(self._h, _vp(b), npairs, n, width, _vp(u), _vp(y), _vp(sh)))
        return y, sh

    def set_device_io(self, on):
        _chk(lib().lgc_ot_sender_set_device_io(self._h, 1 if on else 0))

    def gilboa_ptr(self, b_ptr, npairs, n, width, u_ptr, y_ptr, shares_ptr):
        _chk(lib().lgc_ot_gilboa_send(self._h, C.c_void_p(b_ptr), npairs, n, width, C.c_void_p(u_ptr), C.c_void_p(y_ptr), C.c_void_p(shares_ptr)))

    def gilboa_matrix(self, xs, r, width, u):
        xs = np.ascontiguousarray(xs, dtype=np.uint64); rows, s = xs.shape
        y = np.zeros((rows * r * width, s), dtype=np.uint32 if width == 32 else np.uint64); sh = np.zeros((r, s), dtype=np.uint64)
        _chk(lib().lgc_ot_gilboa_matrix_send(self._h, _vp(xs), rows, r, s, width, _vp(u), _vp(y), _vp(sh)))
        return y, sh

    def gilboa_matrix_ptr(self, xs_ptr, rows, r, s, width, u_ptr, y_ptr, shares_ptr):
        _chk(lib().lgc_ot_gilboa_matrix_send(self._h, C.c_void_p(xs_ptr), rows, r, s, width, C.c_void_p(u_ptr), C.c_void_p(y_ptr),
                                             C.c_void_p(shares_ptr)))

    def gilboa_half(self, xs, r, width, u):
        xs = np.ascontiguousarray(xs, dtype=np.uint64); rows, s = xs.shape
        y = np.zeros((rows * r * (width // 2 + 1), s), dtype=np.uint32 if width == 32 else np.uint64); sh = np.zeros((r, s), dtype=np.uint64)
        _chk(lib().lgc_ot_gilboa_half_send(self._h, _vp(xs), rows, r, s, width, _vp(u), _vp(y), _vp(sh)))
        return y, sh

    def gilboa_half_ptr(self, xs_ptr, rows, r, s, width, u_ptr, y_ptr, shares_ptr):
        _chk(lib().lgc_ot_gilboa_half_send(self._h, C.c_void_p(xs_ptr), rows, r, s, width, C.c_void_p(u_ptr), C.c_void_p(y_ptr),
                                           C.c_void_p(shares_ptr)))

    def labels(self, m0, m1, u):
        m0 = np.ascontiguousarray(m0, dtype=np.uint8).reshape(-1, 16); m1 = np.ascontiguousarray(m1, dtype=np.uint8).reshape(-1, 16)
        e = np.zeros((len(m0), 32), dtype=np.uint8)
        _chk(lib().lgc_ot_labels_send(self._h, _vp(m0), _vp(m1), len(m0), _vp(u), _vp(e)))
        return e

    def close(self):
        if self._h:
            lib().lgc_ot_sender_destroy(self._h); self._h = None

    def __del__(self):
        try:
            self.close()
        except Exception:
            pass


class OtReceiver:

    def __init__(self, seeds0, seeds1, device=0):
        seeds0 = np.ascontiguousarray(seeds0, dtype=np.uint8).reshape(128, 16)
        seeds1 = np.ascontiguousarray(seeds1, dtype=np.uint8).reshape(128, 16)
        self._h = C.c_void_p()
        _chk(lib().lgc_ot_receiver_create(C.byref(self._h), device, _vp(seeds0), _vp(seeds1)))

    def gilboa_start(self, a, width):
        a = np.ascontiguousarray(a, dtype=np.uint64); npairs, n = a.shape
        u = np.zeros(lib().lgc_ot_u_bytes(npairs * n * width), dtype=np.uint8)
        _chk(lib().lgc_ot_gilboa_recv_start(self._h, _vp(a), npairs, n, width, _vp(u)))
        if not hasattr(self, "_nps"):
            self._nps = []
        self._nps.append(npairs)
        return u

    def set_device_io(self, on):
        _chk(lib().lgc_ot_receiver_set_device_io(self._h, 1 if on else 0))

    def gilboa_start_ptr(self, a_ptr, npairs, n, width, u_ptr):
        _chk(lib().lgc_ot_gilboa_recv_start(self._h, C.c_void_p(a_ptr), npairs, n, width, C.c_void_p(u_ptr)))

    def gilboa_finish_ptr(self, y_ptr, shares_ptr):
        _chk(lib().lgc_ot_gilboa_recv_finish(self._h, C.c_void_p(y_ptr), C.c_void_p(shares_ptr)))

    def gilboa_finish(self, y):
        if not getattr(self, "_nps", None):
            sh = np.zeros(1, dtype=np.uint64)
            _chk(lib().lgc_ot_gilboa_recv_finish(self._h, _vp(np.ascontiguousarray(y, dtype=np.uint64)), _vp(sh)))
        sh = np.zeros(self._nps.pop(0), dtype=np.uint64)
        _chk(lib().lgc_ot_gilboa_recv_finish(self._h, _vp(np.ascontiguousarray(y, dtype=np.uint64)), _vp(sh)))
        return sh

    def gilboa_matrix_start(self, xr, s, width):
        xr = np.ascontiguousarray(xr, dtype=np.uint64); rows, r = xr.shape
        u = np.zeros(lib().lgc_ot_u_bytes(rows * r * width), dtype=np.uint8)
        _chk(lib().lgc_ot_gilboa_matrix_recv_start(self._h, _vp(xr), rows, r, s, width, _vp(u)))
        if not hasattr(self, "_mats"):
            self._mats = []
        self._mats.append((r, s, width))
        return u

    def gilboa_matrix_finish(self, y):
        if not getattr(self, "_mats", None):
            raise LgcError(-5, "no matrix Gilboa receive was started on this receiver")
        r, s, width = self._mats[0]
        sh = np.zeros((r, s), dtype=np.uint64)
        rc = lib().lgc_ot_gilboa_matrix_recv_finish(self._h, _vp(np.ascontiguousarray(y, dtype=np.uint32 if width == 32 else np.uint64)), _vp(sh))
        if rc != -5:
            self._mats.pop(0)
        _chk(rc)
        return sh

    def gilboa_matrix_start_ptr(self, xr_ptr, rows, r, s, width, u_ptr):
        _chk(lib().lgc_ot_gilboa_matrix_recv_start(self._h, C.c_void_p(xr_ptr), rows, r, s, width, C.c_void_p(u_ptr)))

    def gilboa_matrix_finish_ptr(self, y_ptr, shares_ptr):
        _chk(lib().lgc_ot_gilboa_matrix_recv_finish(self._h, C.c_void_p(y_ptr), C.c_void_p(shares_ptr)))

    def gilboa_half_start(self, xr, s, width):
        xr = np.ascontiguousarray(xr, dtype=np.uint64); rows, r = xr.shape
        u = np.zeros(lib().lgc_ot_u_bytes(rows * r * width), dtype=np.uint8)
        _chk(lib().lgc_ot_gilboa_half_recv_start(self._h, _vp(xr), rows, r, s, width, _vp(u)))
        if not hasattr(self, "_halves"):
            self._halves = []
        self._halves.append((r, s, width))
        return u

    def gilboa_half_finish(self, y):
        if not getattr(self, "_halves", None):
            raise LgcError(-5, "no half-payload Gilboa receive was started on this receiver")
        r, s, width = self._halves[0]
        sh = np.zeros((r, s), dtype=np.uint64)
        rc = lib().lgc_ot_gilboa_half_recv_finish(self._h, _vp(np.ascontiguousarray(y, dtype=np.uint32 if width == 32 else np.uint64)), _vp(sh))
        if rc != -5:
            self._halves.pop(0)
        _chk(rc)
        return sh

    def gilboa_half_start_ptr(self, xr_ptr, rows, r, s, width, u_ptr):
        _chk(lib().lgc_ot_gilboa_half_recv_start(self._h, C.c_void_p(xr_ptr), rows, r, s, width, C.c_void_p(u_ptr)))

    def gilboa_half_finish_ptr(self, y_ptr, shares_ptr):
        _chk(lib().lgc_ot_gilboa_half_recv_finish(self._h, C.c_void_p(y_ptr), C.c_void_p(shares_ptr)))

    def labels_start(self, choice):
        choice = np.ascontiguousarray(choice, dtype=np.uint8)
        self._m = len(choice)
        u = np.zeros(lib().lgc_ot_u_bytes(self._m), dtype=np.uint8)
        _chk(lib().lgc_ot_labels_recv_start(self._h, _vp(choice), self._m, _vp(u)))
        return u

    def labels_finish(self, e):
        out = np.zeros((self._m, 16), dtype=np.uint8)
        _chk(lib().lgc_ot_labels_recv_finish(self._h, _vp(np.ascontiguousarray(e, dtype=np.uint8)), _vp(out)))
        return out

    def close(self):
        if self._h:
            lib().lgc_ot_receiver_destroy(self._h); self._h = None

    def __del__(self):
        try:
            self.close()
        except Exception:
            pass


def release_cached_memory():
    lib().lgc_release_cached_memory()


def set_split_kernels(garbler=True, evaluator=True):
    lib().lgc_set_split_kernels(int(bool(garbler)), int(bool(evaluator)))


def reference_gate_count(algorithm, width, d, iterations=0):
    L = lib()
    L.lgc_reference_gate_count.argtypes = [C.c_int, C.c_int, C.c_size_t, C.c_int, C.POINTER(C.c_uint64)]
    L.lgc_reference_gate_count.restype = C.c_int
    g = C.c_uint64()
    alg = ALG[algorithm] if isinstance(algorithm, str) else int(algorithm)
    return int(g.value) if L.lgc_reference_gate_count(alg, width, d, iterations, C.byref(g)) == 0 else None


def set_karatsuba(on=True):
    lib().lgc_set_karatsuba.argtypes = [C.c_int]; lib().lgc_set_karatsuba.restype = None
    lib().lgc_set_karatsuba(int(bool(on)))


def set_table_ring_slack(nbytes):
    lib().lgc_set_table_ring_slack.argtypes = [C.c_size_t]; lib().lgc_set_table_ring_slack.restype = None
    lib().lgc_set_table_ring_slack(int(nbytes))




def devices_preflight(devices):
    arr = (C.c_int * len(devices))(*[int(v) for v in devices])
    L = lib()
    L.lgc_devices_preflight.argtypes = [C.c_void_p, C.c_size_t]; L.lgc_devices_preflight.restype = C.c_int
    _chk(L.lgc_devices_preflight(arr, len(devices)))


def gate_hash_eval(labels, tweaks, device=0):
    x = np.ascontiguousarray(labels, dtype=np.uint8).reshape(-1, 16)
    t = np.ascontiguousarray(tweaks, dtype=np.uint64).reshape(-1)
    assert len(t) == len(x)
    out = np.zeros_like(x)
    L = lib()
    L.lgc_gate_hash_eval.argtypes = [C.c_int, C.c_void_p, C.c_void_p, C.c_void_p, C.c_size_t]; L.lgc_gate_hash_eval.restype = C.c_int
    _chk(L.lgc_gate_hash_eval(device, x.ctypes.data, t.ctypes.data, out.ctypes.data, len(x)))
    return out


class RowItem(C.Structure):
    _fields_ = [("label", C.c_uint8 * 16), ("tweak0", C.c_uint64), ("stride", C.c_uint64), ("rows", C.c_uint32),
                ("reserved", C.c_uint32)]


def row_hash_eval(items, device=0):
    arr = (RowItem * max(len(items), 1))()
    total = 0
    for it, (label, tweak0, stride, rows) in zip(arr, items):
        it.label[:] = bytes(label)
        it.tweak0, it.stride, it.rows = int(tweak0), int(stride), int(rows)
        total += int(rows)
    out = np.zeros((total, 2, 64, 16), dtype=np.uint8)
    L = lib()
    L.lgc_row_hash_eval.argtypes = [C.c_int, C.c_void_p, C.c_size_t, C.c_void_p]; L.lgc_row_hash_eval.restype = C.c_int
    _chk(L.lgc_row_hash_eval(device, C.cast(arr, C.c_void_p), len(items), out.ctypes.data))
    return out


def aes_bench(waves=8192, blocks_per_lane=256, device=0):
    rate, chk = C.c_double(), C.c_uint32()
    _chk(lib().lgc_aes_bench(device, waves, blocks_per_lane, C.byref(rate), C.byref(chk)))
    return rate.value, chk.value


def aes_encrypt(blocks, device=0):
    blocks = np.ascontiguousarray(blocks, dtype=np.uint8).reshape(-1, 16)
    out = np.empty_like(blocks)
    _chk(lib().lgc_aes_encrypt(device, blocks.ctypes.data_as(C.c_void_p), out.ctypes.data_as(C.c_void_p), len(blocks)))
    return out


LM = {"auto": 0, "mac": 1, "mack": 2, "wide": 3, "split": 4, "quad2": 5}


class LaunchConstants(C.Structure):
    _fields_ = [("wide_launch", C.c_uint32), ("narrow_mac", C.c_uint32), ("split_max_recs", C.c_uint32),
                ("mac_chunk", C.c_uint32), ("mac_adapt_lo", C.c_uint32)]


def _test_fn(name, restype, argtypes):
    fn = getattr(lib(), name)
    fn.restype, fn.argtypes = restype, argtypes
    return fn


def _modes(v, n):
    if v is None:
        return None
    v = [LM[m] if isinstance(m, str) else int(m) for m in v]
    assert len(v) == n, (len(v), n)
    return (C.c_int * n)(*v)


class RecordProgram(Program):

    def __init__(self, width, precision, records, launch_sizes, modes_g=None, modes_e=None, n_inputs=0, n_words=None,
                 n_reveal=0):
        self._h = C.c_void_p()
        recs = (Record * len(records))(*[Record(*(tuple(r) + (0,))) for r in records])
        sizes = (C.c_uint32 * len(launch_sizes))(*[int(n) for n in launch_sizes])
        nl = len(launch_sizes)
        vp, sz, u32 = C.c_void_p, C.c_size_t, C.c_uint32
        fn = _test_fn("lgc_test_program_create", C.c_int,
                      [C.POINTER(vp), C.c_int, C.c_int, vp, sz, vp, sz, vp, vp, u32, u32, u32])
        _chk(fn(C.byref(self._h), width, precision, C.cast(recs, vp), len(records), C.cast(sizes, vp), nl,
                _modes(modes_g, nl), _modes(modes_e, nl), n_inputs, n_words, n_reveal))
        self.info = ProgramInfo()
        _chk(lib().lgc_program_info_get(self._h, C.byref(self.info)))
        self.system = make_system(0, width, precision, nshares=1)

    def modes(self):
        n = self.info.n_launches
        g = (C.c_int * n)(); e = (C.c_int * n)()
        _chk(_test_fn("lgc_test_launch_modes", C.c_int, [C.c_void_p, C.c_void_p, C.c_void_p, C.c_size_t])(self._h, g, e, n))
        return list(g), list(e)


class RecordSolver(Solver):

    def __init__(self, program, seed=b"\x01" * 16, device=0):
        assert len(seed) == 16
        self._h = C.c_void_p()
        self.system = program.system
        self._adopt(_Request(program.system))
        self.count = None
        self._prog = program
        _chk(_test_fn("lgc_test_solver_create", C.c_int, [C.POINTER(C.c_void_p), C.c_int, C.c_void_p, C.c_char_p])(
            C.byref(self._h), device, program._h, seed))

    def set_inputs(self, values):
        v = np.ascontiguousarray(values, dtype=np.uint64)
        _chk(lib().lgc_solver_set_shares(self._h, v.ctypes.data_as(C.c_void_p)))

    def reveal(self):
        n = self._prog.info.n_reveal
        out = np.zeros(n, dtype=np.uint64)
        _chk(_test_fn("lgc_test_solver_reveal", C.c_int, [C.c_void_p, C.c_void_p, C.c_size_t])(self._h, out.ctypes.data_as(C.c_void_p), n))
        return out


    def word_labels(self, garbler, first, n):
        out = np.zeros((n, 64, 16), dtype=np.uint8)
        fn = _test_fn("lgc_test_solver_read_words", C.c_int, [C.c_void_p, C.c_int, C.c_uint32, C.c_uint32, C.c_void_p])
        _chk(fn(self._h, int(bool(garbler)), first, n, out.ctypes.data_as(C.c_void_p)))
        return out

    def tables(self, launch):
        steps = int(self._prog.launches()[launch]["steps"])
        out = np.zeros((steps, 2, 64, 16), dtype=np.uint8)
        fn = _test_fn("lgc_test_solver_read_tables", C.c_int, [C.c_void_p, C.c_size_t, C.c_void_p, C.c_size_t])
        _chk(fn(self._h, launch, out.ctypes.data_as(C.c_void_p), out.nbytes))
        return out


def launch_shape(mode, garbler, nrec, cus):
    u = C.c_uint32
    v = [u(), u(), u(), u()]
    fn = _test_fn("lgc_test_launch_shape", C.c_int, [C.c_int, C.c_int, u, u] + [C.POINTER(u)] * 4)
    _chk(fn(LM[mode] if isinstance(mode, str) else int(mode), int(bool(garbler)), nrec, cus, *[C.byref(x) for x in v]))
    return tuple(x.value for x in v)


def launch_constants():
    c = LaunchConstants()
    _test_fn("lgc_test_launch_constants", None, [C.POINTER(LaunchConstants)])(C.byref(c))
    return {k: getattr(c, k) for k, _ in LaunchConstants._fields_}
```

Before: 16.81 billion AND-gates/s.

## Add SPLIT2 launch mode packing two records per workgroup with per-record LDS barriers

Adds a SPLIT2 launch mode in which one 1024-thread workgroup runs two records, 8 waves each, instead of one record with 16 waves. Each record half synchronises through an LDS atomic counter barrier in place of the workgroup-wide s_barrier, and the sum-hash state stage is folded into the hash rounds so fewer waves cover all four quarters. To fit two records in LDS, the scratch layout shrinks by aliasing the KS region onto the X region. The mode is picked automatically for non-MAC launches with more records than the SPLIT limit (up to twice that) and long step counts. The intent is to halve the grid and improve CU use for these mid-sized critical-path launches, at the cost of spin-wait barriers and more serial work per wave.

```diff
diff --git a/include/linreg_gc_debug.h b/include/linreg_gc_debug.h
--- a/include/linreg_gc_debug.h
+++ b/include/linreg_gc_debug.h
@@ -77,6 +77,7 @@
 #define LGC_LM_WIDE 3
 #define LGC_LM_SPLIT 4
 #define LGC_LM_QUAD2 5
+#define LGC_LM_SPLIT2 20
 int lgc_test_program_create(lgc_program **out, int width, int precision, const lgc_record *records, size_t n_records,
                             const uint32_t *launch_nrec, size_t n_launches, const int *mode_g, const int *mode_e,
                             uint32_t n_inputs, uint32_t n_words, uint32_t n_reveal);
@@ -86,6 +87,7 @@
 typedef struct {
     uint32_t wide_launch, narrow_mac, split_max_recs;
     uint32_t mac_chunk, mac_adapt_lo;
+    uint32_t split2_min_steps;
 } lgc_test_constants;
 void lgc_test_launch_constants(lgc_test_constants *c);
 int lgc_test_solver_create(lgc_solver **out, int device, const lgc_program *program, const uint8_t seed[16]);
diff --git a/linreg-mpc_amd/csrc/gc_engine.hip b/linreg-mpc_amd/csrc/gc_engine.hip
--- a/linreg-mpc_amd/csrc/gc_engine.hip
+++ b/linreg-mpc_amd/csrc/gc_engine.hip
@@ -728,7 +728,7 @@
 }
 
 static_assert(LGC_LM_AUTO == LM_NONE && LGC_LM_MAC == LM_MAC && LGC_LM_MACK == LM_MACK && LGC_LM_WIDE == LM_WIDE &&
-              LGC_LM_SPLIT == LM_SPLIT && LGC_LM_QUAD2 == LM_QUAD2, "LGC_LM_* must name the LaunchMode values");
+              LGC_LM_SPLIT == LM_SPLIT && LGC_LM_QUAD2 == LM_QUAD2 && LGC_LM_SPLIT2 == LM_SPLIT2, "LGC_LM_* must name the LaunchMode values");
 struct FootprintMachine : PlainBackend {
     uint64_t word_end = 0, slot_end = 0;
     void see(uint32_t id) { if ((uint64_t)id + 1 > word_end) word_end = (uint64_t)id + 1; }
@@ -740,10 +740,10 @@
     void store2(uint32_t lo, uint32_t hi, W) { see(lo); see(hi); }
     void reveal(uint32_t slot, W) { if ((uint64_t)slot + 1 > slot_end) slot_end = (uint64_t)slot + 1; }
 };
-static bool mode_pairs_steps(LaunchMode m) { return m == LM_SPLIT || m == LM_QUAD2; }
+static bool mode_pairs_steps(LaunchMode m) { return m == LM_SPLIT || m == LM_SPLIT2 || m == LM_QUAD2; }
 static const char *mode_name(int m) {
     static const char *const n[] = {"auto", "MAC", "MACK", "WIDE", "SPLIT", "QUAD2"};
-    return m >= 0 && m <= LM_QUAD2 ? n[m] : "?";
+    return m == LM_SPLIT2 ? "SPLIT2" : m >= 0 && m <= LM_QUAD2 ? n[m] : "?";
 }
 
 extern "C" int lgc_test_program_create(lgc_program **out, int width, int precision, const lgc_record *records, size_t n_records,
@@ -764,7 +764,7 @@
     for (size_t i = 0; i < n_launches; i++)
         for (int role = 0; role < 2; role++) {
             const int m = role ? (mode_e ? mode_e[i] : 0) : (mode_g ? mode_g[i] : 0);
-            if (m < LGC_LM_AUTO || m > LGC_LM_QUAD2) return lgc_fail(LGC_EINVAL, "launch %zu: unknown kernel %d", i, m);
+            if (!gc_mode_known(m)) return lgc_fail(LGC_EINVAL, "launch %zu: unknown kernel %d", i, m);
         }
     const Rec *recs = reinterpret_cast<const Rec *>(records);
     for (size_t i = 0; i < n_records; i++) {
@@ -840,7 +840,7 @@
 extern "C" int lgc_test_launch_shape(int mode, int garbler, uint32_t nrec, uint32_t cus, uint32_t *grid, uint32_t *threads,
                                      uint32_t *per_wg, uint32_t *max_threads) {
     if (!grid || !threads || !per_wg || !max_threads) return lgc_fail(LGC_EINVAL, "null argument");
-    if (mode < LGC_LM_MAC || mode > LGC_LM_QUAD2) return lgc_fail(LGC_EINVAL, "unknown kernel %d", mode);
+    if (mode == LGC_LM_AUTO || !gc_mode_known(mode)) return lgc_fail(LGC_EINVAL, "unknown kernel %d", mode);
     if (cus < 1) return lgc_fail(LGC_EINVAL, "cus must be >= 1");
     const LaunchShape sh = gc_launch_shape((LaunchMode)mode, garbler != 0, nrec, cus);
     *grid = sh.grid; *threads = sh.threads; *per_wg = sh.per_wg;
@@ -848,7 +848,7 @@
     case LM_MAC: *max_threads = garbler ? kTpbMacG : kTpbMacE; break;
     case LM_MACK: *max_threads = garbler ? kTpbMackG : kTpbMackE; break;
     case LM_WIDE: *max_threads = kTpbWide; break;
-    case LM_SPLIT: *max_threads = 1024; break;
+    case LM_SPLIT: case LM_SPLIT2: *max_threads = 1024; break;
     default: *max_threads = 256; break;
     }
     return LGC_OK;
@@ -857,6 +857,7 @@
     c->wide_launch = kWideLaunch;
     c->narrow_mac = kNarrowMac;
     c->split_max_recs = kSplitMaxRecs;
+    c->split2_min_steps = kSplit2MinSteps;
     c->mac_chunk = kMacChunk;
     c->mac_adapt_lo = kMacAdaptLo;
 }
diff --git a/linreg-mpc_amd/csrc/gc_kernels.h b/linreg-mpc_amd/csrc/gc_kernels.h
--- a/linreg-mpc_amd/csrc/gc_kernels.h
+++ b/linreg-mpc_amd/csrc/gc_kernels.h
@@ -46,6 +46,14 @@
                                L.step0, R, w, p);
         }
         break;
+    case LM_SPLIT2:
+        if constexpr (PART == 2) {
+            const LaunchShape sh = gc_launch_shape(m, G, L.nrec, gc_num_cus());
+            hipLaunchKernelGGL((gc_split_kernel<G, 2>), dim3(sh.grid), dim3(sh.threads), 0, st, recs + L.first_rec, L.nrec, words, tab, dec,
+                               L.step0, R, w, p);
+        }
+        break;
+    case LM_PAIRED: break;
     case LM_QUAD2:
         if constexpr (PART == 3) {
             const LaunchShape sh = gc_launch_shape(m, G, L.nrec, gc_num_cus());
diff --git a/linreg-mpc_amd/csrc/gc_launch.h b/linreg-mpc_amd/csrc/gc_launch.h
--- a/linreg-mpc_amd/csrc/gc_launch.h
+++ b/linreg-mpc_amd/csrc/gc_launch.h
@@ -35,6 +35,14 @@
 #define GC_SPLIT_MAX_RECS 256
 #endif
 static constexpr uint32_t kSplitMaxRecs = GC_SPLIT_MAX_RECS;
+#ifndef GC_SPLIT2_MIN_STEPS
+#define GC_SPLIT2_MIN_STEPS 400
+#endif
+static constexpr uint32_t kSplit2MinSteps = GC_SPLIT2_MIN_STEPS;
+#ifndef GC_SPLIT2_MAX_RECS
+#define GC_SPLIT2_MAX_RECS (2 * GC_SPLIT_MAX_RECS)
+#endif
+static constexpr uint32_t kSplit2MaxRecs = GC_SPLIT2_MAX_RECS;
 inline std::atomic<int> &gc_split_enabled(bool garbler) {
     static std::atomic<int> on[2] = {{1}, {1}};
     return on[garbler ? 0 : 1];
@@ -78,15 +86,21 @@
     LM_MACK,
     LM_WIDE,
     LM_SPLIT,
-    LM_QUAD2
+    LM_QUAD2,
+    LM_PAIRED = 16,
+    LM_SPLIT2 = LM_SPLIT | LM_PAIRED
 };
-static_assert(LM_QUAD2 < 256, "Launch::force holds a LaunchMode in a byte");
+static_assert(LM_SPLIT2 < 256, "Launch::force holds a LaunchMode in a byte");
+static inline bool gc_mode_known(int m) { return (m >= LM_NONE && m <= LM_QUAD2) || m == LM_SPLIT2; }
 static inline LaunchMode gc_launch_mode(const Launch &L, bool garbler) {
     if (L.nrec == 0) return LM_NONE;
     if (L.force[garbler ? 0 : 1]) return (LaunchMode)L.force[garbler ? 0 : 1];
     if (L.mac_only && L.nrec >= kNarrowMac) return L.mack ? LM_MACK : LM_MAC;
+    const bool split_on = gc_split_enabled(garbler).load(std::memory_order_relaxed) != 0;
+    if (split_on && L.nrec > kSplitMaxRecs && L.nrec <= kSplit2MaxRecs && !L.mac_only && L.steps >= (uint64_t)kSplit2MinSteps * L.nrec)
+        return LM_SPLIT2;
     if (L.nrec >= kWideLaunch) return LM_WIDE;
-    if (L.nrec <= kSplitMaxRecs && gc_split_enabled(garbler).load(std::memory_order_relaxed)) return LM_SPLIT;
+    if (L.nrec <= kSplitMaxRecs && split_on) return LM_SPLIT;
     return LM_QUAD2;
 }
 struct LaunchShape { uint32_t grid, threads, per_wg; };
@@ -107,13 +121,14 @@
         s.threads = s.per_wg * 64;
     } break;
     case LM_SPLIT: s.per_wg = 1; s.threads = 1024; break;
+    case LM_SPLIT2: s.per_wg = 2; s.threads = 1024; break;
     case LM_QUAD2: s.per_wg = 1; s.threads = 256; break;
     default: return s;
     }
     s.grid = (uint32_t)(((uint64_t)nrec + s.per_wg - 1) / s.per_wg);
     return s;
 }
-static inline bool gc_mode_is_crit(LaunchMode m, const Launch &L) { return L.steps != 0 && m == LM_SPLIT; }
+static inline bool gc_mode_is_crit(LaunchMode m, const Launch &L) { return L.steps != 0 && (m == LM_SPLIT || m == LM_SPLIT2); }
 hipError_t gc_launch_tabfill(const Launch &L, const Lbl *stash, Lbl *tab, Lbl R, hipStream_t st);
 #define GC_KERN_DECL(tag)                                                                                                              \
     hipError_t gc_launch_records_##tag(LaunchMode m, const Rec *recs, const Launch &L, Lbl *words, uint64_t *dec, Lbl *tab, Lbl R, int w, \
@@ -127,7 +142,7 @@
     switch (m) {
     case LM_NONE: return hipSuccess;
     case LM_MAC: case LM_MACK: return G ? gc_launch_records_g_0(m, recs, L, words, dec, tab, R, w, p, st) : gc_launch_records_e_0(m, recs, L, words, dec, tab, R, w, p, st);
-    case LM_SPLIT: return G ? gc_launch_records_g_2(m, recs, L, words, dec, tab, R, w, p, st) : gc_launch_records_e_2(m, recs, L, words, dec, tab, R, w, p, st);
+    case LM_SPLIT: case LM_SPLIT2: return G ? gc_launch_records_g_2(m, recs, L, words, dec, tab, R, w, p, st) : gc_launch_records_e_2(m, recs, L, words, dec, tab, R, w, p, st);
     case LM_WIDE: return G ? gc_launch_records_g_1(m, recs, L, words, dec, tab, R, w, p, st) : gc_launch_records_e_1(m, recs, L, words, dec, tab, R, w, p, st);
     default: return G ? gc_launch_records_g_3(m, recs, L, words, dec, tab, R, w, p, st) : gc_launch_records_e_3(m, recs, L, words, dec, tab, R, w, p, st);
     }
@@ -141,7 +156,7 @@
         case LM_NONE: break;
         case LM_MAC: case LM_MACK: need[0] = true; break;
         case LM_WIDE: need[1] = true; break;
-        case LM_SPLIT: need[2] = true; break;
+        case LM_SPLIT: case LM_SPLIT2: need[2] = true; break;
         default: need[3] = true; break;
         }
     }
diff --git a/linreg-mpc_amd/csrc/gc_split.h b/linreg-mpc_amd/csrc/gc_split.h
--- a/linreg-mpc_amd/csrc/gc_split.h
+++ b/linreg-mpc_amd/csrc/gc_split.h
@@ -31,11 +31,12 @@
     kSplitWord = 4 * kSplitPlane,
     kSplitOp = 0,
     kSplitX = 4 * kSplitWord,
-    kSplitKs = 8 * kSplitWord,
-    kSplitGs = 16 * kSplitWord,
-    kSplitDesc = 20 * kSplitWord,
-    kSplitZero = 20 * kSplitWord + 8,
-    kSplitWords = 20 * kSplitWord + 16
+    kSplitKs = kSplitX,
+    kSplitGs = 8 * kSplitWord,
+    kSplitDesc = 12 * kSplitWord,
+    kSplitZero = 12 * kSplitWord + 8,
+    kSplitBar = 12 * kSplitWord + 12,
+    kSplitWords = 12 * kSplitWord + 16
 };
 
 struct SplitDesc {
@@ -53,6 +54,9 @@
     uint32_t *tabw;
     uint64_t launch_step0;
     int wave, lane;
+    __attribute__((address_space(3))) uint32_t *bar;
+    mutable uint32_t epoch;
+    int rec;
 };
 
 __device__ __forceinline__ uint32_t rfl(uint32_t v) { return (uint32_t)__builtin_amdgcn_readfirstlane((int)v); }
@@ -60,6 +64,16 @@
 __device__ __forceinline__ uint32_t ld_u32_global(const uint32_t *p) { return *(const __attribute__((address_space(1))) uint32_t *)p; }
 __device__ __forceinline__ void st_u32_lds(uint32_t *p, uint32_t v) { *(__attribute__((address_space(3))) uint32_t *)p = v; }
 __device__ __forceinline__ uint32_t ld_u32_lds(const uint32_t *p) { return *(const __attribute__((address_space(3))) uint32_t *)p; }
+
+template <int NQ>
+__device__ __forceinline__ void split_barrier(const SplitHashCtx &hc) {
+    if (NQ == 4) { lds_barrier(); return; }
+    hc.epoch += 4u * NQ;
+    asm volatile("s_waitcnt lgkmcnt(0)" ::: "memory");
+    if (hc.lane == 0) __hip_atomic_fetch_add(hc.bar, 1u, __ATOMIC_RELAXED, __HIP_MEMORY_SCOPE_WORKGROUP);
+    while ((int32_t)(rfl(__hip_atomic_load(hc.bar, __ATOMIC_RELAXED, __HIP_MEMORY_SCOPE_WORKGROUP)) - hc.epoch) < 0) {}
+    asm volatile("" ::: "memory");
+}
 
 __device__ __forceinline__ uint32_t *split_row(const SplitHashCtx &hc, int q, uint64_t st) {
     const int gate = 16 * (hc.wave & 3) + (hc.lane >> 2);
@@ -93,16 +107,19 @@
     st_u32_lds(xo, on ? h : 0u);
 }
 
-template <bool GARBLER>
+template <bool GARBLER, int NQ = 4>
 __device__ __forceinline__ void split_hash_phase(const SplitHashCtx &hc, const SplitDesc &d) {
-    const int q = hc.wave >> 2, r = hc.wave & 3;
-    if (d.kind == 1 && q >= 2) return;
+    const int r = hc.wave & 3;
     const int c = hc.lane & 3, gate = 16 * r + (hc.lane >> 2);
     const uint32_t *op = hc.sx + kSplitOp + c * kSplitPlane + gate;
-    const uint32_t a_op = ld_u32_lds(op + (q & ~1) * kSplitWord), b_op = ld_u32_lds(op + (q | 1) * kSplitWord);
-    const uint64_t st = d.step + (uint64_t)(q >> 1);
-    const uint32_t tg = GARBLER ? 0u : ld_u32_global(split_row(hc, q, st));
-    split_hash_core<GARBLER>(hc, q, (q < 2) ? d.act1 : d.act2, st, a_op, b_op, hc.sx + kSplitX + q * kSplitWord, tg);
+#pragma unroll
+    for (int q = hc.wave >> 2; q < 4; q += NQ) {
+        if (d.kind == 1 && q >= 2) return;
+        const uint32_t a_op = ld_u32_lds(op + (q & ~1) * kSplitWord), b_op = ld_u32_lds(op + (q | 1) * kSplitWord);
+        const uint64_t st = d.step + (uint64_t)(q >> 1);
+        const uint32_t tg = GARBLER ? 0u : ld_u32_global(split_row(hc, q, st));
+        split_hash_core<GARBLER>(hc, q, (q < 2) ? d.act1 : d.act2, st, a_op, b_op, hc.sx + kSplitX + q * kSplitWord, tg);
+    }
 }
 
 #ifndef GC_SPLIT_TRACE
@@ -147,7 +164,7 @@
     const int h = 1 << k, hp = h >> 1;
     const int t = ((g >> k) & 1) ? g : ((g + h) & 63);
     if (k == 0) { a0 = opx + t; a1 = opy + t; return; }
-    const lds_u32 *X0 = sx + kSplitKs + ((k & 1) * 4) * kSplitWord + pl, *X1 = X0 + kSplitWord;
+    const lds_u32 *X0 = sx + kSplitKs + ((k & 1) * 2) * kSplitWord + pl, *X1 = X0 + kSplitWord;
     const lds_u32 *Pp = sx + kSplitGs + (((k - 1) & 1) * 2 + 1) * kSplitWord + pl;
     const bool tp = (g >> (k - 1)) & 1;
     const int ti = tp ? t - hp : t;
@@ -161,7 +178,7 @@
     const int h = 1 << k, hp = h >> 1;
     const bool up = (g >> k) & 1;
     const int mb = (g & ~(2 * h - 1)) | (h - 1);
-    const lds_u32 *X0 = sx + kSplitKs + ((k & 1) * 4) * kSplitWord + pl, *X1 = X0 + kSplitWord;
+    const lds_u32 *X0 = sx + kSplitKs + ((k & 1) * 2) * kSplitWord + pl, *X1 = X0 + kSplitWord;
     if (k == 0) {
         b0 = (up ? X0 : opx) + mb;
         b1 = (up ? X1 : opy) + mb;
@@ -251,13 +268,41 @@
     *xo = on ? h : 0u;
 }
 
-template <bool GARBLER, int Q>
+struct SkState { uint32_t a, b, c; };
+template <int Q>
+__device__ __forceinline__ void sk_state_load(SkState &s, const lds_u32 *sx, int k, int g, int pl) {
+    const lds_u32 *opx = sx + kSplitOp + pl, *opy = opx + kSplitWord, *opc = opx + 2 * kSplitWord;
+    const lds_u32 *X0 = sx + kSplitKs + ((k & 1) * 2) * kSplitWord + pl, *X1 = X0 + kSplitWord;
+    const lds_u32 *Gp = sx + kSplitGs + (((k - 1) & 1) * 2) * kSplitWord + pl, *Pp = Gp + kSplitWord;
+    if (Q == 0) {
+        s.a = X0[g]; s.b = X1[g]; s.c = (k == 0) ? opc[g] : Gp[g];
+    } else if (k == 0) {
+        s.a = opx[g]; s.b = opy[g]; s.c = 0u;
+    } else {
+        const int h = 1 << k, hp = h >> 1;
+        const bool gp = ((g >> (k - 1)) & 1) && g >= h;
+        const int gi = gp ? g - hp : g;
+        s.a = (gp ? X0 : Pp)[gi]; s.b = X1[gi]; s.c = 0u;
+    }
+}
+template <int Q>
+__device__ __forceinline__ void sk_state_store(const SkState &s, lds_u32 *sx, int k, int g, int pl) {
+    lds_u32 *Go = sx + kSplitGs + ((k & 1) * 2) * kSplitWord + pl;
+    if (Q == 0) {
+        Go[g] = (k == 0) ? (s.a ^ s.b ^ s.c) : (s.c ^ (((g >> (k - 1)) & 1) ? (s.a ^ s.b) : 0u));
+    } else {
+        const bool gp = k > 0 && ((g >> (k - 1)) & 1) && g >= (1 << k);
+        Go[kSplitWord + g] = (k == 0 || gp) ? (s.a ^ s.b) : s.a;
+    }
+}
+
+template <bool GARBLER, int Q, int NQ = 4>
 __device__ __forceinline__ void split_sk_hash(const SplitHashCtx &hc, int n, uint64_t st, const SkVals *pre) {
     const int r = hc.wave & 3, c = hc.lane & 3, g = 16 * r + (hc.lane >> 2);
     SkTrace tr;
     (void)tr;
 #if GC_SPLIT_TRACE
-    tr.on = GC_SPLIT_TRACE == 1 && blockIdx.x == 0 && (hc.wave == 0 || hc.wave == 4);
+    tr.on = GC_SPLIT_TRACE == 1 && blockIdx.x == 0 && hc.rec == 0 && (hc.wave == 0 || hc.wave == 4);
     tr.w = hc.wave == 4 ? 1 : 0;
     tr.i = tr.on ? g_split_trace_n[tr.w] : 0u;
     SPLIT_STAMP(1)
@@ -279,18 +324,23 @@
     st += 1;
     row += 512;
     SPLIT_STAMP(2)
-    lds_barrier();
+    split_barrier<NQ>(hc);
     SPLIT_STAMP(3)
+    SkState ss;
     auto level = [&](int k, uint32_t &tg) {
         cur = nxt;
         w = sk_load<GARBLER, Q>(cur.ptr);
-        sk_finish<GARBLER, Q>(hc, cur, w, sx + kSplitKs + (((k + 1) & 1) * 4 + Q) * kSplitWord + pl + g, row, tg,
-                              [&](int rnd) { if (rnd >= 2 && rnd < 6) sk_plan_part<GARBLER, Q>(nxt, rnd - 2, sx, k + 1, g, c, pl, plo, n, st + 1); });
+        sk_finish<GARBLER, Q>(hc, cur, w, sx + kSplitKs + (((k + 1) & 1) * 2 + Q) * kSplitWord + pl + g, row, tg,
+                              [&](int rnd) {
+                                  if (rnd >= 2 && rnd < 6) sk_plan_part<GARBLER, Q>(nxt, rnd - 2, sx, k + 1, g, c, pl, plo, n, st + 1);
+                                  if (NQ == 2 && rnd == 6) sk_state_load<Q>(ss, sx, k, g, pl);
+                                  if (NQ == 2 && rnd == 8) sk_state_store<Q>(ss, sx, k, g, pl);
+                              });
         if (!GARBLER) tg = ld_u32_global(row + (k + 2 < L ? 2 * 512 : 0));
         SPLIT_STAMP(5)
         st += 1;
         row += 512;
-        lds_barrier();
+        split_barrier<NQ>(hc);
         SPLIT_STAMP(3)
     };
     int k = 0;
@@ -311,7 +361,7 @@
     for (int k = 0; k < L; k++) {
         if (q == 2) {
             const int h = 1 << k, hp = h >> 1;
-            const lds_u32 *X0 = sx + kSplitKs + ((k & 1) * 4) * kSplitWord + pl, *X1 = X0 + kSplitWord;
+            const lds_u32 *X0 = sx + kSplitKs + ((k & 1) * 2) * kSplitWord + pl, *X1 = X0 + kSplitWord;
             const lds_u32 *Gp = sx + kSplitGs + (((k - 1) & 1) * 2) * kSplitWord + pl, *Pp = Gp + kSplitWord;
             lds_u32 *Go = sx + kSplitGs + ((k & 1) * 2) * kSplitWord + pl;
             const uint32_t x0 = X0[g], x1 = X1[g];
@@ -333,7 +383,7 @@
     }
 }
 
-template <bool GARBLER>
+template <bool GARBLER, int NQ = 4>
 struct SplitBackend {
     typedef uint32_t W;
     static const bool kPairSteps = true;
@@ -408,29 +458,29 @@
         publish(0, a);
         publish(1, b);
         post(d);
-        lds_barrier();
-        split_hash_phase<GARBLER>(hc, d);
-        lds_barrier();
+        split_barrier<NQ>(hc);
+        split_hash_phase<GARBLER, NQ>(hc, d);
+        split_barrier<NQ>(hc);
         return bit(act) ? (result(0) ^ result(1)) : 0u;
     }
     __device__ __forceinline__ void AND2(W a1, W b1, uint64_t act1, W a2, W b2, uint64_t act2, W &c1, W &c2) {
         SplitDesc d = {2u, act1, act2, step};
         step += 2;
-        if (wave == 0) { SPLIT_STAMP2(0, 6) }
+        if (wave == 0 && hc.rec == 0) { SPLIT_STAMP2(0, 6) }
         publish(0, a1);
         publish(1, b1);
         publish(2, a2);
         publish(3, b2);
         post(d);
-        lds_barrier();
-        if (wave == 0) { SPLIT_STAMP2(0, 7) }
-        split_hash_phase<GARBLER>(hc, d);
-        if (wave == 0) { SPLIT_STAMP2(0, 8) }
-        lds_barrier();
-        if (wave == 0) { SPLIT_STAMP2(0, 9) }
+        split_barrier<NQ>(hc);
+        if (wave == 0 && hc.rec == 0) { SPLIT_STAMP2(0, 7) }
+        split_hash_phase<GARBLER, NQ>(hc, d);
+        if (wave == 0 && hc.rec == 0) { SPLIT_STAMP2(0, 8) }
+        split_barrier<NQ>(hc);
+        if (wave == 0 && hc.rec == 0) { SPLIT_STAMP2(0, 9) }
         c1 = bit(act1) ? (result(0) ^ result(1)) : 0u;
         c2 = bit(act2) ? (result(2) ^ result(3)) : 0u;
-        if (wave == 0) { asm volatile("" :: "v"(c1), "v"(c2)); SPLIT_STAMP2(0, 10) }
+        if (wave == 0 && hc.rec == 0) { asm volatile("" :: "v"(c1), "v"(c2)); SPLIT_STAMP2(0, 10) }
     }
     __device__ __forceinline__ W add_native(W x, W y, int n, W cinw, W *cout) {
         const int L = sk_levels(n);
@@ -441,11 +491,11 @@
         publish(1, y);
         publish(2, cinw);
         post(d, n);
-        lds_barrier();
-        split_sk_hash<GARBLER, 0>(hc, n, st0, (const SkVals *)0);
+        split_barrier<NQ>(hc);
+        split_sk_hash<GARBLER, 0, NQ>(hc, n, st0, (const SkVals *)0);
         const lds_u32 *sx = hc.sxl;
         const int pl = wave * kSplitPlane;
-        const lds_u32 *X0 = sx + kSplitKs + ((L & 1) * 4) * kSplitWord + pl, *X1 = X0 + kSplitWord;
+        const lds_u32 *X0 = sx + kSplitKs + ((L & 1) * 2) * kSplitWord + pl, *X1 = X0 + kSplitWord;
         const lds_u32 *Gp = (L == 0) ? (sx + kSplitOp + 2 * kSplitWord + pl) : (sx + kSplitGs + (((L - 1) & 1) * 2) * kSplitWord + pl);
         const int tm = (lane - 1) & 63;
         const bool xm = (L == 0) || ((tm >> (L - 1)) & 1);
@@ -462,29 +512,38 @@
     __device__ __forceinline__ void finish() {
         SplitDesc d = {0u, 0ull, 0ull, 0ull};
         post(d);
-        lds_barrier();
+        split_barrier<NQ>(hc);
     }
 };
 
-template <bool GARBLER>
+template <bool GARBLER, int NQ = 4>
 __global__ void __launch_bounds__(1024)
 gc_split_kernel(const Rec *recs, uint32_t nrec, Lbl *words, Lbl *tab, uint64_t *decode, uint64_t launch_step0, Lbl R, int w, int p) {
+    constexpr int kRecs = 4 / NQ, kRecThreads = 1024 / kRecs;
+    static_assert(NQ == 4 || NQ == 2, "16 or 8 waves per record");
+    static_assert((2 * kLdsTabWords + 2 * kSplitWords) * 4 <= 160 * 1024 && kSplitWords % 4 == 0, "LDS of the two-record form");
     __shared__ uint32_t lds_te0[2 * kLdsTabWords];
-    __shared__ __attribute__((aligned(16))) uint32_t lds_sx[kSplitWords];
+    __shared__ __attribute__((aligned(16))) uint32_t lds_sx_all[kRecs * kSplitWords];
+    const int rec = (NQ == 4) ? 0 : __builtin_amdgcn_readfirstlane(threadIdx.x / kRecThreads);
+    uint32_t *lds_sx = lds_sx_all + rec * kSplitWords;
+    if (NQ == 2 && threadIdx.x % kRecThreads == 0) { lds_sx[kSplitZero] = 0u; lds_sx[kSplitBar] = 0u; }
     lds_tab4_fill(lds_te0);
-    const uint32_t wid = blockIdx.x;
+    const uint32_t wid = blockIdx.x * kRecs + rec;
     if (wid >= nrec) return;
     SplitHashCtx hc;
     hc.lt = lds_tab4_make(lds_te0);
     hc.lane = threadIdx.x & 63;
-    hc.wave = __builtin_amdgcn_readfirstlane(threadIdx.x >> 6);
+    hc.wave = __builtin_amdgcn_readfirstlane((threadIdx.x % kRecThreads) >> 6);
+    hc.rec = rec;
     const int c = hc.lane & 3;
 #pragma unroll
     for (int k = 0; k < 11; k++) hc.rkl[k] = c_aes.rk[4 * k + c];
     hc.Rq = GARBLER ? (c == 0 ? R.x : c == 1 ? R.y : c == 2 ? R.z : R.w) : 0u;
     hc.sx = lds_sx;
     hc.sxl = (__attribute__((address_space(3))) uint32_t *)lds_sx;
-    if (threadIdx.x == 0) lds_sx[kSplitZero] = 0u;
+    hc.bar = hc.sxl + kSplitBar;
+    hc.epoch = 0u;
+    if (NQ == 4 && threadIdx.x == 0) lds_sx[kSplitZero] = 0u;
     hc.tabw = reinterpret_cast<uint32_t *>(tab);
     hc.launch_step0 = launch_step0;
     if (hc.wave >= 4) {
@@ -494,11 +553,11 @@
         sk_ptrs_own<1>(first1, hc.sxl, -1, g_, pl_);
         sk_ptrs_oth<1>(first1, hc.sxl, -1, g_, GARBLER ? 0 : pl_);
         for (;;) {
-            lds_barrier();
+            split_barrier<NQ>(hc);
             typedef const __attribute__((address_space(3))) gc_u32x4 *lds4;
             const gc_u32x4 lo = ((lds4)(lds_sx + kSplitDesc))[0];
             SkVals pre;
-            if (q == 1) pre = sk_load<GARBLER, 1>(first1);
+            if (NQ == 2 || q == 1) pre = sk_load<GARBLER, 1>(first1);
             SplitDesc d;
             const uint32_t kn = rfl(lo.x);
             d.kind = kn & 0xffu;
@@ -506,21 +565,21 @@
             d.step = ((uint64_t)rfl(lo.z) << 32) | rfl(lo.y);
             if (d.kind == 3u) {
                 const int n = (int)(kn >> 8);
-                if (q == 1) split_sk_hash<GARBLER, 1>(hc, n, d.step, &pre);
+                if (NQ == 2 || q == 1) split_sk_hash<GARBLER, 1, NQ>(hc, n, d.step, &pre);
                 else split_sk_side(hc, n);
                 continue;
             }
             const gc_u32x4 hi = ((lds4)(lds_sx + kSplitDesc))[1];
             d.act1 = ((uint64_t)rfl(hi.x) << 32) | rfl(lo.w);
             d.act2 = ((uint64_t)rfl(hi.z) << 32) | rfl(hi.y);
-            if (hc.wave == 4) { SPLIT_STAMP2(1, 7) }
-            split_hash_phase<GARBLER>(hc, d);
-            if (hc.wave == 4) { SPLIT_STAMP2(1, 8) }
-            lds_barrier();
-            if (hc.wave == 4) { SPLIT_STAMP2(1, 9) }
+            if (hc.wave == 4 && rec == 0) { SPLIT_STAMP2(1, 7) }
+            split_hash_phase<GARBLER, NQ>(hc, d);
+            if (hc.wave == 4 && rec == 0) { SPLIT_STAMP2(1, 8) }
+            split_barrier<NQ>(hc);
+            if (hc.wave == 4 && rec == 0) { SPLIT_STAMP2(1, 9) }
         }
     }
-    SplitBackend<GARBLER> be;
+    SplitBackend<GARBLER, NQ> be;
     be.hc = hc;
     be.wave = hc.wave;
     be.lane = hc.lane;
diff --git a/linreg-mpc_amd/python/linreg_gc.py b/linreg-mpc_amd/python/linreg_gc.py
--- a/linreg-mpc_amd/python/linreg_gc.py
+++ b/linreg-mpc_amd/python/linreg_gc.py
@@ -1240,12 +1240,12 @@
     return out
 
 
-LM = {"auto": 0, "mac": 1, "mack": 2, "wide": 3, "split": 4, "quad2": 5}
+LM = {"auto": 0, "mac": 1, "mack": 2, "wide": 3, "split": 4, "quad2": 5, "split2": 20}
 
 
 class LaunchConstants(C.Structure):
     _fields_ = [("wide_launch", C.c_uint32), ("narrow_mac", C.c_uint32), ("split_max_recs", C.c_uint32),
-                ("mac_chunk", C.c_uint32), ("mac_adapt_lo", C.c_uint32)]
+                ("mac_chunk", C.c_uint32), ("mac_adapt_lo", C.c_uint32), ("split2_min_steps", C.c_uint32)]
 
 
 def _test_fn(name, restype, argtypes):
```

Measured after the change: 17.04 billion AND-gates/s (median of 6 runs). 1.4% higher.
